# jhuldr/BrainFM

Measured on AMD Instinct MI355X. Metric: voxels/sec whole-volume multi-task inference, 256^3 tiled, higher is better.
Workload: dtype f16x3-split (fp32-grade); 1 GPU; 256^3 volume, reference tiling win160/stride80 -> 27 tiles, UNet3D f64 x6 levels, 9 heads (69 ch), fused tail + deformed atlas + on-device stitch of 17 keys; stitched_keys=17, mfma_passes=3, submission=hipGraph replay per tile shape, parallelism=tiles sharded over 1 rank(s), gather to rank 0, tiles_in_flight_per_gpu=2

## Files before the change

### brainfm_amd/_lib.py

```python
import ctypes as C
import os

_HERE = os.path.dirname(os.path.abspath(__file__))
LIB_PATH = os.path.join(_HERE, "libbrainfm_hip.so")

ERR = {0: "BFM_OK", -1: "BFM_E_ARG", -2: "BFM_E_SHAPE", -3: "BFM_E_WORKSPACE", -4: "BFM_E_LAUNCH"}

ROLE_PLAIN, ROLE_CT, ROLE_BIAS_LOG, ROLE_SEG, ROLE_DIST, ROLE_SR, ROLE_PATHOL = range(7)
(EW_EXP, EW_AFFINE, EW_CLAMP, EW_CLAMP_MIN, EW_GAMMA, EW_SIGMOID, EW_DIV, EW_NONZERO, EW_SUB_DIV, EW_GE,
 EW_NAN_TO_NUM) = range(11)
(EW_ADD, EW_MUL, EW_MUL_EXP, EW_AXPY_CLAMP0, EW_AXPY, EW_DIV2, EW_ZERO_WHERE_ZERO) = range(7)


class BfmError(RuntimeError):
    pass


class Upsample(C.Structure):
    _fields_ = [("d", C.c_int), ("h", C.c_int), ("w", C.c_int),
                ("mapD", C.c_void_p), ("mapH", C.c_void_p), ("mapW", C.c_void_p),
                ("repD", C.c_void_p), ("repH", C.c_void_p), ("repW", C.c_void_p)]


CLASS_STATS_BLOCKS = 1024


class TailDesc(C.Structure):
    _fields_ = [("n_out", C.c_int), ("c_feat", C.c_int),
                ("head_w", C.c_void_p), ("head_b", C.c_void_p), ("roles", C.c_void_p), ("out_slot", C.c_void_p),
                ("seg_first", C.c_int), ("n_seg", C.c_int), ("seg_lut", C.c_void_p),
                ("n_dist", C.c_int), ("dist_first", C.c_int), ("max_dist", C.c_float),
                ("unit_feat", C.c_int), ("slot_high_res", C.c_int), ("slot_fake_cortical", C.c_int),
                ("n_maps", C.c_int), ("head_wmax", C.c_float), ("skip_zero_input", C.c_int)]


class ZoomAxis(C.Structure):
    _fields_ = [("f", C.c_void_p), ("c", C.c_void_p), ("wf", C.c_void_p), ("wc", C.c_void_p)]


class KSet(C.Structure):
    _fields_ = [("k", C.c_void_p * 7), ("coef", C.c_float * 7), ("nk", C.c_int)]


class Dopri5Advect(C.Structure):
    _fields_ = [("y", C.c_void_p * 2), ("f", C.c_void_p * 2), ("k", C.c_void_p * 5),
                ("Vx", C.c_void_p), ("Vy", C.c_void_p), ("Vz", C.c_void_p),
                ("sx", C.c_int), ("sy", C.c_int), ("sz", C.c_int), ("neumann_bc", C.c_int), ("is_f64", C.c_int),
                ("atol", C.c_double), ("rtol", C.c_double), ("tol_min_dt", C.c_double), ("dt_max", C.c_double),
                ("safety", C.c_double), ("ifactor", C.c_double), ("dfactor", C.c_double),
                ("t_out", C.c_void_p), ("nt", C.c_int), ("sol", C.c_void_p), ("state", C.c_void_p),
                ("workspace", C.c_void_p)]


class AgeParams(C.Structure):
    _fields_ = [(n, C.c_void_p) for n in ("c1w", "c1b", "c2w", "c2b", "l1w", "l1b", "l2w", "l2b", "l3w", "l3b")]


class AgeGrads(C.Structure):
    _fields_ = [(n, C.c_void_p) for n in ("c1w", "c1b", "c2w", "c2b", "l1w", "l1b", "l2w", "l2b", "l3w", "l3b")]


GATHER_MAX_JOBS = 12


VERTEX_SETS_MAX = 4


class VertexSet(C.Structure):
    _fields_ = [("V", C.c_void_p), ("n", C.c_int64)]


class GatherJob(C.Structure):
    _fields_ = [("src", C.c_void_p), ("out", C.c_void_p), ("mean", C.c_float), ("scale", C.c_float), ("pre", C.c_int),
                ("default_max", C.c_int), ("post_div", C.c_float), ("clamp", C.c_int), ("clamp_lo", C.c_float),
                ("clamp_hi", C.c_float), ("sign", C.c_float), ("want_minmax", C.c_int)]


_P = C.c_void_p
_I = C.c_int
_F = C.c_float
_L = C.c_int64
_Z = C.c_size_t
_UP = C.POINTER(Upsample)

SIGNATURES = {
    "bfm_version": (C.c_char_p, []),
    "bfm_gn_stats_workspace": (_Z, [_I, _I, _I, _I, _I, _UP]),
    "bfm_gn_stats": (_I, [_P, _I, _P, _I, _I, _I, _I, _UP, _P, _P, _I, _F, _P, _P, _P, _P, _Z, _P]),
    "bfm_pack_conv_weights_direct": (_I, [_P, _I, _I, _P, _P]),
    "bfm_pack_conv_weights_mfma_bytes": (_Z, [_I, _I]),
    "bfm_pack_conv_weights_mfma": (_I, [_P, _I, _I, _F, _P, C.POINTER(_I), _P]),
    "bfm_pack_conv_weights_mfma16_bytes": (_Z, [_I, _I]),
    "bfm_pack_conv_weights_mfma16": (_I, [_P, _I, _I, _F, _P, C.POINTER(_I), _P]),
    "bfm_conv3x3x3_direct": (_I, [_P, _I, _P, _I, _I, _I, _I, _UP, _P, _P, _P, _I, _F, _P, _P]),
    "bfm_pack_conv_weights_upfold_bytes": (C.c_size_t, [_I, _I, _I]),
    "bfm_pack_conv_weights_upfold": (_I, [_P, _I, _I, _I, _F, _I, _P, _P, _P]),
    "bfm_conv3x3x3_upfold": (_I, [_P, _I, _I, _I, _I, _P, _P, _P, _I, _P, _I, _I, _I, _P, _P]),
    "bfm_conv3x3x3_upfold_workspace": (_Z, [_I, _I, _I, _I, _I]),
    "bfm_conv3x3x3_upfold_ex": (_I, [_P, _I, _I, _I, _I, _P, _P, _P, _I, _P, _I, _I, _I, _P, _P, _Z, _P]),
    "bfm_conv3x3x3_upfold_batch_workspace": (_Z, [_I, _I, _I, _I, _I, _I]),
    "bfm_conv3x3x3_upfold_batch": (_I, [_P, _I, _I, _I, _I, _I, _P, _P, _P, _I, _P, _I, _I, _I, _P, _P, _Z, _I, _P]),
    "bfm_moment_rows_bytes": (_Z, [_I, _I]),
    "bfm_conv3x3x3_mfma_rows": (_I, [_I, _I, _I, _I, _I, C.POINTER(_I)]),
    "bfm_conv3x3x3_mfma_ex": (_I, [_P, _I, _P, _I, _I, _I, _I, _UP, _P, _P, _P, _I, _P, _I, _I, _F, _I,
                                   C.POINTER(_I), _P, _P, _Z, _P, _P]),
    "bfm_conv3x3x3_mfma_batch_workspace": (_Z, [_I, _I, _I, _I, _I, _I, _I]),
    "bfm_conv3x3x3_mfma_batch": (_I, [_P, _I, _P, _I, _I, _I, _I, _I, _UP, _P, _P, _P, _I, _P, _I, _I, _F, _I,
                                      C.POINTER(_I), _P, _P, _Z, _P, _I, _P]),
    "bfm_gn_stats_batch_workspace": (_Z, [_I, _I, _I, _I, _I, _I, _UP]),
    "bfm_gn_stats_batch": (_I, [_P, _I, _P, _I, _I, _I, _I, _I, _UP, _P, _P, _I, _F, _P, _P, _P, _P, _Z, _P]),
    "bfm_gn_stats_rows_batch": (_I, [_P, _I, _I, _P, _I, _I, C.c_double, _L, _I, _P, _P, _I, _F, _P, _P, _P, _P]),
    "bfm_conv3x3x3_stem_rows": (_I, [_I, _I, _I]),
    "bfm_conv3x3x3_stem_ex": (_I, [_P, _I, _I, _I, _P, _P, _P, _P, _I, _F, _P, _P, _P]),
    "bfm_conv3x3x3_stem_mc_ex": (_I, [_P, _I, _I, _I, _I, _P, _P, _P, _P, _I, _F, _P, _P, _P]),
    "bfm_gn_stats_rows_workspace": (_Z, [_I, _I, _I, _I]),
    "bfm_gn_stats_rows": (_I, [_P, _I, _I, _P, _I, _I, C.c_double, _L, _P, _P, _I, _F, _P, _P, _P, _P, _Z, _P, _P]),
    "bfm_gn_stats_rows_sliced": (_I, [_P, _I, _I, _I, _I, _P, _I, _I, _I, _I, C.c_double, _L, _P, _P, _I, _F, _P, _P, _P, _P, _Z,
                                      _P, _P]),
    "bfm_gn_stats_rows_train": (_I, [_P, _I, _I, _P, _I, _I, C.c_double, _L, _P, _P, _I, _F, _P, _P, _P, _P, _P, _P, _Z, _P, _P]),
    "bfm_crop3d": (_I, [_P, _I, _I, _I, _I, _I, _I, _I, _I, _I, _P, _P]),
    "bfm_pack_conv_weights_wino4_bytes": (_Z, [_I, _I, _I]),
    "bfm_pack_conv_weights_wino4": (_I, [_P, _I, _I, _F, _I, _P, C.POINTER(_I), _P]),
    "bfm_conv3x3x3_wino4_rows": (_I, [_I, _I, _I, _I]),
    "bfm_conv3x3x3_wino4_box": (_I, [_I, _I, _I, _I, _P]),
    "bfm_conv3x3x3_wino4_masked_workspace": (_Z, [_I, _I, _I, _I]),
    "bfm_conv3x3x3_wino4_uniform_scratch": (_Z, [_I]),
    "bfm_conv3x3x3_wino4_uniform": (_I, [_P, _I, _I, _I, _I, _P, _P, _P, _I, _P, _I, _I, _F, _I, _I, _P, _P, _P, _P, _P]),
    "bfm_conv3x3x3_wino4": (_I, [_P, _I, _I, _I, _I, _P, _P, _P, _I, _P, _I, _I, _F, _I, _I, _P, _P, _P]),
    "bfm_conv3x3x3_wino4_batch": (_I, [_P, _I, _I, _I, _I, _I, _P, _P, _P, _I, _P, _I, _I, _F, _I, _I, _P, _P, _I, _P]),
    "bfm_conv3x3x3_wino4_masked": (_I, [_P, _I, _I, _I, _I, _P, _P, _P, _I, _P, _I, _I, _F, _I, _I, _P, _P, _P, _Z, _P]),
    "bfm_permute_flip3d": (_I, [_P, _I, _I, _I, C.POINTER(_I), C.POINTER(_I), _P, _P]),
    "bfm_bbox_nonzero": (_I, [_P, _I, _I, _I, _F, _P, _P]),
    "bfm_mean_lastdim": (_I, [_P, _L, _I, _P, _P]),
    "bfm_pack_conv_weights_wino_bytes": (_Z, [_I, _I, _I]),
    "bfm_pack_conv_weights_wino": (_I, [_P, _I, _I, _F, _I, _P, C.POINTER(_I), _P]),
    "bfm_bspline3_prefilter_axis": (_I, [_P, _I, _I, _I, _I, _I, _F, _F, _P, _F, _F, _F, _P]),
    "bfm_bspline3_resample_axis": (_I, [_P, _I, _I, _I, _I, _P, _I, _I, _P, _P]),
    "bfm_conv3x3x3_wino_rows": (_I, [_I, _I, _I, _I]),
    "bfm_conv3x3x3_wino_ex": (_I, [_P, _I, _I, _I, _I, _P, _P, _P, _I, _P, _I, _I, _F, _I, _I, _P, _P, _P]),
    "bfm_conv3x3x3_wino_box": (_I, [_I, _I, _I, _I, _P]),
    "bfm_uniform_boxes": (_I, [_P, _I, _I, _I, _I, _I, _P, _P]),
    "bfm_uniform_boxes_level": (_I, [_P, _I, _I, _I, _I, _I, _I, _P, _P]),
    "bfm_uniform_boxes_bytes": (_Z, [_I, _I, _I, _I]),
    "bfm_conv3x3x3_wino_uniform_scratch": (_Z, [_I]),
    "bfm_conv3x3x3_wino_uniform": (_I, [_P, _I, _I, _I, _I, _P, _P, _P, _I, _P, _I, _I, _F, _I, _I, _P, _P, _P, _P, _P]),
    "bfm_conv3x3x3_wino_pool_ok": (_I, [_I, _I, _I, _I]),
    "bfm_conv3x3x3_wino_pool": (_I, [_P, _I, _I, _I, _I, _P, _P, _P, _I, _P, _I, _I, _F, _I, _I, _P, _P, _P, _P, _P]),
    "bfm_conv3x3x3_wino_uniform_pool": (_I, [_P, _I, _I, _I, _I, _P, _P, _P, _I, _P, _I, _I, _F, _I, _I, _P, _P, _P, _P, _P, _P,
                                             _P]),
    "bfm_conv3x3x3_wino_masked_workspace": (_Z, [_I, _I, _I, _I]),
    "bfm_conv3x3x3_wino_masked": (_I, [_P, _I, _I, _I, _I, _P, _P, _P, _I, _P, _I, _I, _F, _I, _I, _P, _P, _P, _Z, _P]),
    "bfm_maxpool2_rows": (_I, [_I, _I, _I, _I]),
    "bfm_maxpool2_ex": (_I, [_P, _I, _I, _I, _I, _P, _P, _P]),
    "bfm_maxpool2_batch_rows": (_I, [_I, _I, _I, _I]),
    "bfm_maxpool2_batch": (_I, [_P, _I, _I, _I, _I, _I, _P, _P, _P]),
    "bfm_grid_push3d_linear": (_I, [_P, _I, _I, _I, _I, _I, _P, _I, _I, _I, _I, C.POINTER(_I), _I, _P, _P]),
    "bfm_grid_grad3d_linear": (_I, [_P, _I, _I, _I, _I, _I, _P, _I, _I, _I, _I, C.POINTER(_I), _I, _P, _P]),
    "bfm_gn_stats_train": (_I, [_P, _I, _P, _I, _I, _I, _I, _UP, _P, _P, _I, _F, _P, _P, _P, _P, _P, _P, _Z, _P]),
    "bfm_lrelu_bwd": (_I, [_P, _P, _L, _F, _P, _P]),
    "bfm_lrelu_bwd_ex": (_I, [_P, _P, _L, _F, _P, _P, _P]),
    "bfm_conv3x3x3_wgrad_workspace": (_Z, [_I, _I, _I, _I, _I]),
    "bfm_conv3x3x3_wgrad": (_I, [_P, _I, _P, _I, _P, _I, _I, _I, _I, _UP, _P, _P, _P, _P, _Z, _P]),
    "bfm_conv3x3x3_wgrad_ex": (_I, [_P, _I, _P, _I, _P, _I, _I, _I, _I, _UP, _P, _P, _P, _P, _I, _I, _P, _P, _Z, _P]),
    "bfm_stem_mc_bwd_workspace": (_Z, [_I, _I, _I, _I, _I]),
    "bfm_stem_mc_bwd": (_I, [_P, _I, _P, _I, _I, _I, _I, _P, _P, _P, _P, _P, _P, _P, _P, _P, _Z, _P]),
    "bfm_gn_bwd_workspace": (_Z, [_I, _I, _I, _I]),
    "bfm_gn_bwd": (_I, [_P, _P, _I, _P, _I, _I, _I, _I, _UP, _P, _P, _P, _P, _P, _P, _I, _P, _P, _P, _P, _P, _Z, _P]),
    "bfm_maxpool2_bwd": (_I, [_P, _P, _I, _I, _I, _I, _P, _P]),
    "bfm_transpose_mirror_weights": (_I, [_P, _I, _I, _I, _P, _P]),
    "bfm_loss_workspace": (_Z, [_I]),
    "bfm_loss_l1": (_I, [_P, _I, _I, _P, _P, _P, _L, _F, _I, _F, _P, _P, _P, _Z, _P]),
    "bfm_loss_l1_multi_workspace": (_Z, []),
    "bfm_loss_l1_multi": (_I, [_P, _I, _L, _I, _P, _P, _P, _P, _P, _P, _P, _P, _P, _P, _Z, _P]),
    "bfm_loss_grad_l1_multi": (_I, [_P, _I, _I, _P, _P, _P, _P, _I, _I, _I, _P, _P, _P, _Z, _P]),
    "bfm_loss_grad_l1": (_I, [_P, _I, _I, _P, _P, _I, _I, _I, _F, _P, _P, _P, _Z, _P]),
    "bfm_loss_seg": (_I, [_P, _I, _I, _I, _P, _P, _P, _L, _F, _F, _P, _P, _P, _P, _Z, _P]),
    "bfm_loss_pathol_workspace": (_Z, []),
    "bfm_loss_pathol": (_I, [_P, _L, _L, _P, _L, _F, _F, _P, _P, _P, _P, _Z, _P]),
    "bfm_loss_reg_workspace": (_Z, [_I, _I, _I, _I]),
    "bfm_loss_reg_smooth": (_I, [_P, _L, _L, _L, _I, _I, _I, _I, _F, _P, _P, _P, _Z, _P]),
    "bfm_loss_reg_hessian": (_I, [_P, _L, _L, _L, _I, _I, _I, _I, _F, _P, _P, _P, _Z, _P]),
    "bfm_loss_contrastive_workspace": (_Z, []),
    "bfm_loss_contrastive": (_I, [_P, _P, _I, _L, _I, _F, _F, _F, _F, _F, _P, _P, _P, _P, _P, _P, _Z, _P]),
    "bfm_head_bwd_workspace": (_Z, [_I, _I, _L]),
    "bfm_head_bwd": (_I, [_P, _P, _P, _I, _I, _L, _P, _P, _P, _P, _Z, _P]),
    "bfm_tail_raw_rows": (_I, [_P, _L, C.POINTER(TailDesc), _P, _P, _L, _P]),
    "bfm_loss_l1_multi_rows": (_I, [_P, _L, _I, _L, _I, _P, _P, _P, _P, _P, _P, _P, _P, _P, _P, _Z, _P]),
    "bfm_loss_grad_l1_multi_rows": (_I, [_P, _L, _I, _I, _P, _P, _P, _P, _I, _I, _I, _P, _P, _P, _Z, _P]),
    "bfm_loss_seg_rows": (_I, [_P, _L, _I, _I, _I, _P, _P, _P, _L, _F, _F, _P, _P, _P, _P, _Z, _P]),
    "bfm_head_bwd_rows": (_I, [_P, _L, _P, _P, _I, _I, _L, _P, _P, _P, _P, _Z, _P]),
    "bfm_normalize_bwd": (_I, [_P, _P, _I, _L, _F, _P, _P]),
    "bfm_adamw_step": (_I, [_P, _P, _P, _P, _L, _F, _F, _F, _F, _F, _I, _F, _P]),
    "bfm_grad_sumsq": (_I, [_P, _L, _P, _P, _P, _Z, _P]),
    "bfm_grad_sumsq_multi": (_I, [_P, _I, _P, _I, _L, _P, _P, _P, _Z, _P]),
    "bfm_adamw_step_multi": (_I, [_P, _I, _P, _I, _L, _F, _F, _F, _F, _F, _P]),
    "bfm_conv3x3x3_mfma_workspace": (_Z, [_I, _I, _I, _I, _I, _I]),
    "bfm_conv3x3x3_mfma_plan": (_I, [_I, _I, _I, _I, _I, C.POINTER(_I)]),
    "bfm_conv3x3x3_mfma": (_I, [_P, _I, _P, _I, _I, _I, _I, _UP, _P, _P, _P, _I, _P, _I, _I, _F, _I,
                                C.POINTER(_I), _P, _P, _Z, _P]),
    "bfm_maxpool2": (_I, [_P, _I, _I, _I, _I, _P, _P]),
    "bfm_tail_heads": (_I, [_P, _P, _L, C.POINTER(TailDesc), _P, _P, _P, _P, _P, _P]),
    "bfm_tail_heads_rows": (_I, [_P, _P, _L, C.POINTER(TailDesc), _P, _P, _L, _P, _P, _I, _P]),
    "bfm_ew_unary": (_I, [_I, _P, _L, _P, _L, _L, _F, _F, _P]),
    "bfm_ew_binary": (_I, [_I, _P, _L, _P, _L, _P, _L, _L, _F, _P]),
    "bfm_absmax_f32": (_I, [_P, _L, _L, _L, _P, _P]),
    "bfm_softmax_cl": (_I, [_P, _L, _I, _P, _L, _L, _P]),
    "bfm_argmax_lut_cl": (_I, [_P, _L, _I, _P, _P, _L, _P]),
    "bfm_fake_cortical": (_I, [_P, _L, _I, _P, _L, _P]),
    "bfm_mask_concat2": (_I, [_P, _P, _L, _P, _P]),
    "bfm_condition_input": (_I, [_P, _P, _I, _I, _I, _I, _P, _P, _P, _P]),
    "bfm_interp3d_linear": (_I, [_P, _I, _I, _I, _I, _P, _P, _P, _L, _F, _P, _P]),
    "bfm_interp3d_nearest": (_I, [_P, _I, _I, _I, _I, _P, _P, _P, _L, _P, _P]),
    "bfm_deformed_atlas": (_I, [_P, _P, _P, _P, _P, _I, _I, _I, C.POINTER(_F), _L, _P, _P]),
    "bfm_deformed_atlas_tile": (_I, [_P, _P, _P, _P, _P, _I, _I, _I, C.POINTER(_F), _L, _P, _P]),
    "bfm_zoom_linear": (_I, [_P, _I, _I, _I, _I, C.POINTER(ZoomAxis), _I, _I, _I, _P, _P]),
    "bfm_conv1d_axis": (_I, [_P, _I, _I, _I, _I, _P, _I, _P, _P]),
    "bfm_grid_pull3d_linear": (_I, [_P, _I, _I, _I, _I, _I, _P, _I, _I, _I, _I, C.POINTER(_I), _I, _P, _P]),
    "bfm_deform_grid_workspace": (_Z, [_I, _I, _I]),
    "bfm_deform_grid": (_I, [_P, _I, _I, _I, C.POINTER(_F), C.POINTER(_F), C.POINTER(_I), _P, _P, _P, _P, _P, _Z, _P]),
    "bfm_label_gauss": (_I, [_P, _P, _P, _P, _L, _I, _P, _P]),
    "bfm_label_class_stats": (_I, [_P, _P, _L, _P, _P, _P, _P]),
    "bfm_onehot_lut": (_I, [_P, _P, _I, _I, _L, _P, _P]),
    "bfm_perlin3d": (_I, [_P, _I, _I, _I, _I, _I, _I, _P, _P]),
    "bfm_radix_hist_f64": (_I, [_P, _L, C.c_uint64, _I, _P, _P]),
    "bfm_threshold_mask_f64": (_I, [_P, _L, C.c_double, _P, _P, _P]),
    "bfm_curl3d": (_I, [_P, _P, _P, _I, _I, _I, _F, _P, _P, _P, _P]),
    "bfm_advect_upwind_rhs": (_I, [_P, _I, _P, _P, _P, _I, _I, _I, _I, _P, _P]),
    "bfm_rk_combine": (_I, [_P, _I, C.POINTER(KSet), _P, _L, _P]),
    "bfm_reduce_workspace": (_Z, []),
    "bfm_rk_error_sumsq": (_I, [C.POINTER(KSet), _P, _P, _I, C.c_double, C.c_double, _L, _P, _P, _Z, _P]),
    "bfm_scaled_sumsq": (_I, [_P, _P, _I, _P, _I, C.c_double, C.c_double, _L, _P, _P, _Z, _P]),
    "bfm_dopri5_dense_eval": (_I, [_P, _P, _I, C.POINTER(KSet), C.c_double, C.c_double, _P, _L, _P]),
    "bfm_reduce_f32": (_I, [_I, _P, _P, _L, _P, _P, _Z, _P]),
    "bfm_reduce_f64": (_I, [_I, _P, _P, _L, _P, _P, _Z, _P]),
    "bfm_dopri5_advect_state_bytes": (_Z, []),
    "bfm_dopri5_advect_workspace": (_Z, [_I, _I, _I]),
    "bfm_dopri5_advect_init": (_I, [C.POINTER(Dopri5Advect), C.c_double, C.c_double, _P]),
    "bfm_dopri5_advect_steps": (_I, [C.POINTER(Dopri5Advect), _I, _P]),
    "bfm_randn_philox": (_I, [_P, _L, C.c_uint64, C.c_uint64, _F, _P]),
    "bfm_svf_integrate_workspace": (_Z, [_I, _I, _I]),
    "bfm_svf_integrate": (_I, [_P, _I, _I, _I, _I, _P, _P, _P, _Z, _P]),
    "bfm_deform_vertices": (_I, [_P, _I, _I, _I, C.POINTER(VertexSet), _I, C.POINTER(_F), C.POINTER(_F), _I, _I, _P]),
    "bfm_deform_zoom_workspace": (_Z, []),
    "bfm_deform_zoom_minmax": (_I, [_P, _I, _I, _I, C.POINTER(ZoomAxis), _I, _I, _I, _I, C.POINTER(_F), C.POINTER(_F),
                                    C.POINTER(_I), _P, _P, _Z, _P]),
    "bfm_deform_zoom_write": (_I, [_P, _I, _I, _I, C.POINTER(ZoomAxis), _I, _I, _I, _I, C.POINTER(_F), C.POINTER(_F),
                                   C.POINTER(_I), C.POINTER(_F), _P, _P, _P, _P, _P]),
    "bfm_gather_targets_workspace": (_Z, []),
    "bfm_gather_targets": (_I, [C.POINTER(GatherJob), _I, _I, _I, _I, C.POINTER(_I), _P, _P, _P, _I, _I, _I, _I, _P, _P,
                                _Z, _P]),
    "bfm_minmax_normalise": (_I, [_P, _L, _P, _P]),
    "bfm_gather_onehot": (_I, [_P, _I, _I, _I, C.POINTER(_I), _P, _P, _P, _I, _I, _I, _I, _P, _I, _I, _P, _P, _P]),
    "bfm_gather_onehot_rows": (_I, [_P, _I, _I, _I, C.POINTER(_I), _P, _P, _P, _I, _I, _I, _I, _P, _I, _I, _P, _P, _P]),
    "bfm_percentile_workspace": (_Z, []),
    "bfm_percentile_f64": (_I, [_P, _L, _L, _I, C.c_double, _P, _P, _Z, _P]),
    "bfm_shape_workspace": (_Z, []),
    "bfm_shape_threshold_f64": (_I, [_P, _L, _P, _P, _P, _P, _P, _Z, _P]),
    "bfm_shape_binarize": (_I, [_P, _I, _L, _P, C.c_double, _P, _P, _P, _Z, _P]),
    "bfm_pathology_mask": (_I, [_P, _P, _I, _P, _L, _P, _P, _Z, _P]),
    "bfm_pathology_encode_workspace": (_Z, []),
    "bfm_pathology_encode_dev": (_I, [_P, _P, _P, _I, _P, C.POINTER(_F), _I, _P, _L, _P, _P, _P, _Z, _P]),
    "bfm_interp3d_linear_axes": (_I, [_P, _I, _I, _I, _P, _P, _P, _I, _I, _I, _F, _P, _P]),
    "bfm_sample_finalize": (_I, [_P, _P, _I, _I, _I, _P, _I, _P, _P, _P]),
    "bfm_stitch_accumulate": (_I, [_P, _P, _P, _I, _I, _I, _P, _I, _I, _I, _I, _I, _I, _P]),
    "bfm_stitch_accumulate_multi": (_I, [_P, _L, _P, _I, _P, _P, _I, _I, _I, _P, _I, _I, _I, _I, _I, _I, _P]),
    "bfm_tile_count_add": (_I, [_P, _I, _I, _I, _I, _I, _I, _I, _I, _I, _P]),
    "bfm_pack_tile_multi": (_I, [_P, _L, _P, _I, _P, _P, _L, _P, _P]),
    "bfm_divide_by_count_multi": (_I, [_P, _P, _L, _I, _P]),
    "bfm_stitch_gather_multi": (_I, [_P, _I, _I, _P, _I, _I, _I, _P]),
    "bfm_tile_mask_blocks": (_I, [_L]),
    "bfm_tile_mask_index": (_I, [_P, _I, _I, _I, _P, _I, _I, _P, _P, _P, _P]),
    "bfm_pack_tile_compact": (_I, [_P, _L, _P, _I, _P, _P, _L, _P, _L, _P, _P]),
    "bfm_stitch_gather_compact": (_I, [_P, _I, _I, _P, _P, _I, _I, _I, _P]),
    "bfm_maxpool4": (_I, [_P, _I, _I, _I, _I, _P, _P, _P]),
    "bfm_maxpool4_bwd": (_I, [_P, _P, _I, _I, _I, _I, _P, _I, _P]),
    "bfm_age_conv_fwd": (_I, [_P, _I, _I, _I, _I, _P, _P, _I, _P, _P]),
    "bfm_age_conv_bwd_workspace": (_Z, [_I, _I, _I, _I, _I]),
    "bfm_age_conv_bwd": (_I, [_P, _I, _I, _I, _I, _P, _I, _P, _P, _P, _P, _P, _P, _Z, _P]),
    "bfm_age_mlp_fwd": (_I, [_P, _I, C.POINTER(AgeParams), _I, _P, _P, _P, _P]),
    "bfm_age_mlp_bwd_workspace": (_Z, []),
    "bfm_age_mlp_bwd": (_I, [_P, _I, C.POINTER(AgeParams), _I, _P, _P, _P, _P, C.c_double, _F, _P, C.POINTER(AgeGrads),
                             _P, _P, _Z, _P]),
}

_lib = None


def register(sigs):
    SIGNATURES.update(sigs)
    if _lib is not None:
        _bind(_lib, sigs)


def _bind(lib, sigs):
    for name, (res, args) in sigs.items():
        try:
            fn = getattr(lib, name)
        except AttributeError as e:
            raise BfmError("libbrainfm_hip.so does not export %s -- rebuild it" % name) from e
        fn.restype = res
        fn.argtypes = args


def load():
    global _lib
    if _lib is None:
        if not os.path.exists(LIB_PATH):
            raise BfmError("HIP extension missing: %s (run `python -m brainfm_amd.build`); "
                           "there is no CPU fallback in the product path" % LIB_PATH)
        import torch
        lib = C.CDLL(LIB_PATH)
        _bind(lib, SIGNATURES)
        _lib = lib
    return _lib


def check(rc, what):
    if rc != 0:
        raise BfmError("%s failed: %s (%d)" % (what, ERR.get(rc, "?"), rc))


def ptr(t):
    if t is None:
        return None
    return C.c_void_p(t.data_ptr())


def stream_ptr():
    import torch
    raw = getattr(torch._C, "_cuda_getCurrentRawStream", None)
    if raw is not None:
        return C.c_void_p(raw(torch._C._cuda_getDevice()))
    return C.c_void_p(torch.cuda.current_stream().cuda_stream)


def on_device(pick):
    import functools

    def deco(fn):
        @functools.wraps(fn)
        def wrapped(*a, **k):
            import torch
            d = pick(*a, **k)
            if isinstance(d, torch.Tensor):
                d = d.device
            if isinstance(d, int):
                d = torch.device("cuda", d)
            if isinstance(d, str):
                d = torch.device(d)
            if d is None or d.type != "cuda" or d.index is None or d.index == torch.cuda.current_device():
                return fn(*a, **k)
            with torch.cuda.device(d):
                return fn(*a, **k)
        return wrapped
    return deco
```

### brainfm_amd/csrc/conv3d_mfma.hip

```cpp
#include "conv_shared.h"
#include <cstdlib>
#include <type_traits>

namespace {

typedef _Float16 half8 __attribute__((ext_vector_type(8)));
typedef _Float16 half4 __attribute__((ext_vector_type(4)));
typedef float floatx16 __attribute__((ext_vector_type(16)));

constexpr int KC = 16;
#ifdef BFM_STAMPS
__device__ long long g_stamps[4096];
#define STAMP(i) do { if (stamp_on) g_stamps[stamp_base + (i)] = clock64(); } while (0)
#else
#define STAMP(i) do {} while (0)
#endif
constexpr int FRAG_U4 = 64;

struct ConvParams {
    const float *A, *B;
    int CA, CB, D, H, W;
    UpView up;
    const float *scale, *shift, *bound;
    int G;
    const uint4* wp;
    int wexp;
    int Cout;
    float slope;
    float* out;
    int TD, TH, TW, HT, WT;
    int nTy, nTx, nMt, NT;
    int KCN, kc_per_split, splitk;
    int nvox_lds, plane_stride;
    int tw_shift, thw_shift;
    int64_t split_stride;
    int accum;
    int S, nMtS;
    int saff;
    int64_t sA, sB, sO;
    double *rsum, *rsq;
    float *rmn, *rmx;
    int abl;
};


template <int WM, int WN>
__device__ __forceinline__ void store_moment_row(const ConvParams& p, unsigned char* lds, int tid, int wm, int wn,
                                                 bool writer, const int (&col)[4], int ncol, const double (&s)[4],
                                                 const double (&q)[4], const float (&mn)[4], const float (&mx)[4],
                                                 int mt, int nt) {
    double* ls = reinterpret_cast<double*>(lds);
    double* lq = ls + WM * WN * 64;
    float* lmn = reinterpret_cast<float*>(lq + WM * WN * 64);
    float* lmx = lmn + WM * WN * 64;
    __syncthreads();
    if (writer) {
#pragma unroll
        for (int j = 0; j < 4; ++j) {
            if (j < ncol) {
                const int i = (wm * WN + wn) * 64 + col[j];
                ls[i] = s[j]; lq[i] = q[j]; lmn[i] = mn[j]; lmx[i] = mx[j];
            }
        }
    }
    __syncthreads();
    if (tid < 64 * WN) {
        const int w2 = tid >> 6, c = tid & 63;
        double S = 0.0, Q = 0.0;
        float MN = INFINITY, MX = -INFINITY;
#pragma unroll
        for (int m = 0; m < WM; ++m) {
            const int i = (m * WN + w2) * 64 + c;
            S += ls[i]; Q += lq[i];
            MN = fminf(MN, lmn[i]); MX = fmaxf(MX, lmx[i]);
        }
        const size_t o = (size_t)mt * p.Cout + (nt * WN + w2) * 64 + c;
        p.rsum[o] = S; p.rsq[o] = Q; p.rmn[o] = MN; p.rmx[o] = MX;
    }
}

__device__ __forceinline__ void box_coords(const ConvParams& p, int q, int& d, int& h, int& w) {
    if (p.tw_shift >= 0 && p.thw_shift >= 0) {
        d = q >> p.thw_shift;
        int rem = q & ((1 << p.thw_shift) - 1);
        h = rem >> p.tw_shift;
        w = rem & ((1 << p.tw_shift) - 1);
    } else {
        int thw = p.TH * p.TW;
        d = q / thw;
        int rem = q - d * thw;
        h = rem / p.TW;
        w = rem - h * p.TW;
    }
}

template <int ROWS, int NTHR>
__device__ __forceinline__ const int* build_row_table(const ConvParams& p, unsigned char* lds, int tid, int z0, int y0, int x0,
                                                      int boxN) {
    int* tab = reinterpret_cast<int*>(lds);
    for (int q = tid; q < ROWS; q += NTHR) {
        int rel = -1;
        if (q < boxN) {
            int d, h, w;
            box_coords(p, q, d, h, w);
            if (z0 + d < p.D && y0 + h < p.H && x0 + w < p.W) rel = ((d * p.H + h) * p.W + w) * p.Cout;
        }
        tab[q] = rel;
    }
    return tab;
}

template <int WM, int WN, int NPASS, int NSLOT>
__global__ void __launch_bounds__(64 * WM * WN, 2) conv_mfma(const ConvParams p) {
    constexpr int NTHR = 64 * WM * WN;
    constexpr int NW = WM * WN;
    constexpr int NPL = (NPASS == 3) ? 2 : 1;
    constexpr int ROWFR = 12 * WN;
    constexpr int KPR = ROWFR / NW;
    constexpr int DPF = NSLOT - 1;
    static_assert(ROWFR % NW == 0, "row fragments must split evenly over the waves");
    extern __shared__ __attribute__((aligned(16))) unsigned char lds[];

    const int tid = threadIdx.x;
    const int lane = tid & 63;
    const int wave = __builtin_amdgcn_readfirstlane(tid >> 6);
    const int wm = wave / WN, wn = wave % WN;
    const int l32 = lane & 31, khalf = lane >> 5;

    int bid = blockIdx.x;
    {
        const int nblk = p.nMt * p.NT;
        const int q = nblk >> 3, r = nblk & 7;
        const int xcd = bid & 7, idx = bid >> 3;
        bid = (xcd < r ? xcd * (q + 1) : r * (q + 1) + (xcd - r) * q) + idx;
    }
    int mt, nt, smp = 0;
    if (p.S > 1) {
        smp = bid % p.S;
        const int t = bid / p.S;
        nt = t % p.NT;
        mt = smp * p.nMtS + t / p.NT;
    } else {
        mt = bid / p.NT;
        nt = bid - mt * p.NT;
    }
    const int mtl = mt - smp * p.nMtS;
    const float* const pA = p.A + smp * p.sA;
    const float* const pB = p.B + smp * p.sB;
    const float* const pscale = p.scale + smp * p.saff;
    const float* const pshift = p.shift + smp * p.saff;
    const float* const pbound = p.bound + smp * p.G;
    float* const pout = p.out + smp * p.sO;
    const int split = blockIdx.y;
#ifdef BFM_STAMPS
    const bool stamp_on = tid == 0 && (blockIdx.x == 0 || blockIdx.x == gridDim.x / 2 + 3) && blockIdx.y == gridDim.y / 2;
    int stamp_base = blockIdx.x == 0 ? 0 : 1024;
    long long t_wait = 0, t_bar = 0;
#endif
    const int tx = mtl % p.nTx;
    const int ty = (mtl / p.nTx) % p.nTy;
    const int tz = mtl / (p.nTx * p.nTy);
    const int z0 = tz * p.TD, y0 = ty * p.TH, x0 = tx * p.TW;
    const int boxN = p.TD * p.TH * p.TW;

    float bmax = 0.f;
    for (int g = 0; g < p.G; ++g) bmax = fmaxf(bmax, pbound[g]);
    int aexp = 0;
    if (bmax > 0.f && bmax < INFINITY) {
        int ex;
        (void)frexpf(bmax, &ex);
        aexp = 14 - ex;
        aexp = aexp > 60 ? 60 : (aexp < -60 ? -60 : aexp);
    }
    const float a_scale = ldexpf(1.0f, aexp);
    const float dq = ldexpf(1.0f, -(aexp + p.wexp));

    int a_off[2];
#pragma unroll
    for (int mb = 0; mb < 2; ++mb) {
        int q = wm * 64 + mb * 32 + row_perm(l32);
        int d = 0, h = 0, w = 0;
        if (q < boxN) box_coords(p, q, d, h, w);
        int vox = (d * p.HT + h) * p.WT + w;
        a_off[mb] = (khalf * NPL) * p.plane_stride + vox * 16;
    }

    constexpr int MAX_IT = 12;
    const int n_el = p.nvox_lds * 4;
    const int q4 = tid & 3;
    int off[MAX_IT];
    auto compute_offsets = [&](bool fromB) {
#pragma unroll
        for (int it = 0; it < MAX_IT; ++it) {
            const int e = tid + it * NTHR;
            off[it] = -2;
            if (e < n_el) {
                const int vox = e >> 2;
                const int hz = vox / (p.HT * p.WT);
                const int rem = vox - hz * (p.HT * p.WT);
                const int hy = rem / p.WT;
                const int hx = rem - hy * p.WT;
                const int gz = z0 + hz - 1, gy = y0 + hy - 1, gx = x0 + hx - 1;
                off[it] = -1;
                if (gz >= 0 && gz < p.D && gy >= 0 && gy < p.H && gx >= 0 && gx < p.W) {
                    if (fromB) off[it] = ((p.up.mapD[gz] * p.up.h + p.up.mapH[gy]) * p.up.w + p.up.mapW[gx]) * p.CB;
                    else off[it] = ((gz * p.H + gy) * p.W + gx) * p.CA;
                }
            }
        }
    };
    bool off_fromB = (split * p.kc_per_split * KC) >= p.CA;
    compute_offsets(off_fromB);
    const int st_plane = ((q4 >> 1) * NPL) * p.plane_stride + (q4 & 1) * 8;

    floatx16 acc[2][2];
#pragma unroll
    for (int mb = 0; mb < 2; ++mb)
#pragma unroll
        for (int nb = 0; nb < 2; ++nb)
#pragma unroll
            for (int i = 0; i < 16; ++i) acc[mb][nb][i] = 0.f;

    const int ntw = nt * WN + wn;
    if (p.accum && p.splitk == 1) {
        const float inv_dq = ldexpf(1.0f, aexp + p.wexp);
        const int* rowtab = build_row_table<WM * 64, NTHR>(p, lds, tid, z0, y0, x0, boxN);
        __syncthreads();
        const float* ib = pout + (((int64_t)z0 * p.H + y0) * p.W + x0) * p.Cout + ntw * 64 + l32;
#pragma unroll
        for (int mb = 0; mb < 2; ++mb) {
#pragma unroll
            for (int ig = 0; ig < 4; ++ig) {
                const int4 r4 = *reinterpret_cast<const int4*>(rowtab + wm * 64 + mb * 32 + row_perm(ig * 8 + khalf * 4));
                const int rel[4] = {r4.x, r4.y, r4.z, r4.w};
#pragma unroll
                for (int j = 0; j < 4; ++j) {
                    if (rel[j] < 0) continue;
                    const float* orow = ib + (unsigned)rel[j];
#pragma unroll
                    for (int nb = 0; nb < 2; ++nb) acc[mb][nb][ig * 4 + j] = orow[nb * 32] * inv_dq;
                }
            }
        }
    }
    const int kc_begin = split * p.kc_per_split;
    int kc_end = min(p.KCN, kc_begin + p.kc_per_split);
#ifdef BFM_MFMA_ABLATE
    if (p.abl & 32) kc_end = kc_begin;
#endif

    const int b_base = 2 * NPL * p.plane_stride;
    const int total_rows = (kc_end - kc_begin) * 9;
    auto issue_row = [&](int R) {
        const int Rc = R < total_rows ? R : total_rows - 1;
        const int kcR = kc_begin + Rc / 9, rr = Rc % 9;
        const int slot = R % NSLOT;
#pragma unroll
        for (int i = 0; i < KPR; ++i) {
            const int f = wave + i * NW;
            const int j = f / 12, g = f - j * 12;
            const uint4* src = p.wp + ((size_t)((nt * WN + j) * p.KCN + kcR) * 27 + rr * 3) * (4 * FRAG_U4) +
                               g * FRAG_U4 + lane;
            __builtin_amdgcn_global_load_lds((const __attribute__((address_space(1))) void*)src,
                                             (__attribute__((address_space(3))) void*)(lds + b_base +
                                                                                      (slot * ROWFR + f) * 1024),
                                             16, 0, 0);
        }
    };
    if (total_rows > 0) {
#pragma unroll
        for (int R = 0; R < DPF; ++R) issue_row(R);
    }

    for (int kc = kc_begin; kc < kc_end; ++kc) {
        const int c0 = kc * KC;
        const bool fromB = c0 >= p.CA;
        if (fromB != off_fromB) { off_fromB = fromB; compute_offsets(fromB); }
        const float* src = (fromB ? pB + (c0 - p.CA) : pA + c0) + q4 * 4;
        const float4 sc4 = *reinterpret_cast<const float4*>(pscale + c0 + q4 * 4);
        const float4 sh4 = *reinterpret_cast<const float4*>(pshift + c0 + q4 * 4);
        const float sc[4] = {sc4.x * a_scale, sc4.y * a_scale, sc4.z * a_scale, sc4.w * a_scale};
        const float sh[4] = {sh4.x * a_scale, sh4.y * a_scale, sh4.z * a_scale, sh4.w * a_scale};

        STAMP((kc - kc_begin) * 8 + 0);
        __syncthreads();
        STAMP((kc - kc_begin) * 8 + 1);
#pragma unroll
        for (int it0 = 0; it0 < MAX_IT; it0 += 4) {
            float4 v[4];
#pragma unroll
            for (int u = 0; u < 4; ++u) {
                v[u] = make_float4(0.f, 0.f, 0.f, 0.f);
                if (off[it0 + u] >= 0) v[u] = *reinterpret_cast<const float4*>(src + off[it0 + u]);
            }
#pragma unroll
            for (int u = 0; u < 4; ++u) {
                const int e = tid + (it0 + u) * NTHR;
                if (off[it0 + u] != -2) {
                    const bool ok = off[it0 + u] >= 0;
                    float y[4] = {v[u].x, v[u].y, v[u].z, v[u].w};
                    half4 hi, lo;
#pragma unroll
                    for (int i = 0; i < 4; ++i) {
                        float t = ok ? fmaf(y[i], sc[i], sh[i]) : 0.f;
                        _Float16 hh = (_Float16)t;
                        hi[i] = hh;
                        lo[i] = (_Float16)(t - (float)hh);
                    }
                    unsigned char* dst = lds + st_plane + (e >> 2) * 16;
                    *reinterpret_cast<half4*>(dst) = hi;
                    if constexpr (NPASS == 3) *reinterpret_cast<half4*>(dst + p.plane_stride) = lo;
                }
            }
        }
        STAMP((kc - kc_begin) * 8 + 2);
        __syncthreads();
        STAMP((kc - kc_begin) * 8 + 3);

        const int rbase = (kc - kc_begin) * 9;
        for (int r = 0; r < 9; ++r) {
            const int R = rbase + r;
#ifdef BFM_STAMPS
            long long ta = 0, tb = 0, tc = 0;
            if (stamp_on) ta = clock64();
#endif
            asm volatile("s_waitcnt vmcnt(%0)" ::"n"(KPR * (DPF - 1)) : "memory");
#ifdef BFM_STAMPS
            if (stamp_on) tb = clock64();
#endif
            __builtin_amdgcn_s_barrier();
#ifdef BFM_STAMPS
            if (stamp_on) { tc = clock64(); t_wait += tb - ta; t_bar += tc - tb; }
#endif
            issue_row(R + DPF);
            const unsigned char* bs = lds + b_base + ((R % NSLOT) * ROWFR + wn * 12) * 1024 + lane * 16;
            const int kd = r / 3, kh = r - kd * 3;
            const int roff = (kd * p.HT + kh) * p.WT * 16;
#pragma unroll
            for (int kw = 0; kw < 3; ++kw) {
                half8 a[2][NPL], b[2][NPL];
#pragma unroll
                for (int nb = 0; nb < 2; ++nb)
#pragma unroll
                    for (int hl = 0; hl < NPL; ++hl)
                        b[nb][hl] = *reinterpret_cast<const half8*>(bs + (kw * 4 + nb * 2 + hl) * 1024);
#pragma unroll
                for (int mb = 0; mb < 2; ++mb)
#pragma unroll
                    for (int hl = 0; hl < NPL; ++hl)
                        a[mb][hl] = *reinterpret_cast<const half8*>(lds + a_off[mb] + hl * p.plane_stride + roff +
                                                                    kw * 16);
#pragma unroll
                for (int mb = 0; mb < 2; ++mb)
#pragma unroll
                    for (int nb = 0; nb < 2; ++nb) {
                        if constexpr (NPASS == 3) {
                            acc[mb][nb] = __builtin_amdgcn_mfma_f32_32x32x16_f16(a[mb][1], b[nb][0], acc[mb][nb], 0, 0, 0);
                            acc[mb][nb] = __builtin_amdgcn_mfma_f32_32x32x16_f16(a[mb][0], b[nb][1], acc[mb][nb], 0, 0, 0);
                        }
                        acc[mb][nb] = __builtin_amdgcn_mfma_f32_32x32x16_f16(a[mb][0], b[nb][0], acc[mb][nb], 0, 0, 0);
                    }
            }
        }
    }
    asm volatile("s_waitcnt vmcnt(0)" ::: "memory");
#ifdef BFM_STAMPS
    if (stamp_on) { g_stamps[stamp_base + 1000] = t_wait; g_stamps[stamp_base + 1001] = t_bar; g_stamps[stamp_base + 1002] = clock64();
                    g_stamps[stamp_base + 1003] = kc_end - kc_begin; }
#endif

#ifdef BFM_MFMA_ABLATE
    if (p.abl & 16) {
        float sm = 0.f;
#pragma unroll
        for (int mb = 0; mb < 2; ++mb)
#pragma unroll
            for (int i = 0; i < 16; ++i) sm += acc[mb][0][i] + acc[mb][1][i];
        if (sm == 12345.678f) pout[tid] = sm;
        return;
    }
#endif
    const bool final_out = p.splitk == 1;
    const bool want_rows = final_out && p.rsum != nullptr;
    float* obase = pout + (final_out ? 0 : (int64_t)split * p.split_stride);
    float fs[4] = {0.f, 0.f, 0.f, 0.f}, fq[4] = {0.f, 0.f, 0.f, 0.f};
    float mmn[4] = {INFINITY, INFINITY, INFINITY, INFINITY}, mmx[4] = {-INFINITY, -INFINITY, -INFINITY, -INFINITY};
    __syncthreads();
    const int* rowtab = build_row_table<WM * 64, NTHR>(p, lds, tid, z0, y0, x0, boxN);
    __syncthreads();
    float* const ob = obase + (((int64_t)z0 * p.H + y0) * p.W + x0) * p.Cout + ntw * 64 + l32;
#pragma unroll
    for (int mb = 0; mb < 2; ++mb) {
#pragma unroll
        for (int ig = 0; ig < 4; ++ig) {
            const int4 r4 = *reinterpret_cast<const int4*>(rowtab + wm * 64 + mb * 32 + row_perm(ig * 8 + khalf * 4));
            const int rel[4] = {r4.x, r4.y, r4.z, r4.w};
#pragma unroll
            for (int j = 0; j < 4; ++j) {
                if (rel[j] < 0) continue;
                float* orow = ob + (unsigned)rel[j];
#pragma unroll
                for (int nb = 0; nb < 2; ++nb) {
                    float r = acc[mb][nb][ig * 4 + j] * dq;
                    if (final_out) r = r >= 0.f ? r : r * p.slope;
                    orow[nb * 32] = r;
                    if (want_rows) {
                        fs[nb] += r; fq[nb] = fmaf(r, r, fq[nb]);
                        mmn[nb] = fminf(mmn[nb], r); mmx[nb] = fmaxf(mmx[nb], r);
                    }
                }
            }
        }
    }
    if (want_rows) {
        double ms[4], mq[4];
#pragma unroll
        for (int j = 0; j < 4; ++j) { ms[j] = (double)fs[j]; mq[j] = (double)fq[j]; }
#pragma unroll
        for (int nb = 0; nb < 2; ++nb) {
            ms[nb] += __shfl_xor(ms[nb], 32);
            mq[nb] += __shfl_xor(mq[nb], 32);
            mmn[nb] = fminf(mmn[nb], __shfl_xor(mmn[nb], 32));
            mmx[nb] = fmaxf(mmx[nb], __shfl_xor(mmx[nb], 32));
        }
        const int cols[4] = {l32, 32 + l32, 0, 0};
        store_moment_row<WM, WN>(p, lds, tid, wm, wn, khalf == 0, cols, 2, ms, mq, mmn, mmx, mt, nt);
    }
}

template <int WM, int WN, int NPASS, int SP, int NSLOT>
__global__ void __launch_bounds__(64 * WM * WN, 2) conv_mfma16(const ConvParams p) {
    constexpr int NTHR = 64 * WM * WN;
    constexpr int NW = WM * WN;
    constexpr int NPL = (NPASS == 3) ? 2 : 1;
    constexpr int PAIRFR = 8 * WN;
    constexpr int SLOTFR = SP * PAIRFR;
    constexpr int KPS = SLOTFR / NW;
    constexpr int NSL = 14 / SP;
    constexpr int DPF = NSLOT - 1;
    static_assert(SLOTFR % NW == 0 && 14 % SP == 0, "slot geometry");
    typedef float floatx4 __attribute__((ext_vector_type(4)));
    extern __shared__ __attribute__((aligned(16))) unsigned char lds[];

    const int tid = threadIdx.x;
    const int lane = tid & 63;
    const int wave = __builtin_amdgcn_readfirstlane(tid >> 6);
    const int wm = wave / WN, wn = wave % WN;
    const int l16 = lane & 15, kg = lane >> 4;

    int bid = blockIdx.x;
    {
        const int nblk = p.nMt * p.NT;
        const int q = nblk >> 3, r = nblk & 7;
        const int xcd = bid & 7, idx = bid >> 3;
        bid = (xcd < r ? xcd * (q + 1) : r * (q + 1) + (xcd - r) * q) + idx;
    }
    int mt, nt, smp = 0;
    if (p.S > 1) {
        smp = bid % p.S;
        const int t = bid / p.S;
        nt = t % p.NT;
        mt = smp * p.nMtS + t / p.NT;
    } else {
        mt = bid / p.NT;
        nt = bid - mt * p.NT;
    }
    const int mtl = mt - smp * p.nMtS;
    const float* const pA = p.A + smp * p.sA;
    const float* const pB = p.B + smp * p.sB;
    const float* const pscale = p.scale + smp * p.saff;
    const float* const pshift = p.shift + smp * p.saff;
    const float* const pbound = p.bound + smp * p.G;
    float* const pout = p.out + smp * p.sO;
    const int split = blockIdx.y;
    const int tx = mtl % p.nTx;
    const int ty = (mtl / p.nTx) % p.nTy;
    const int tz = mtl / (p.nTx * p.nTy);
    const int z0 = tz * p.TD, y0 = ty * p.TH, x0 = tx * p.TW;
    const int boxN = p.TD * p.TH * p.TW;

    float bmax = 0.f;
    for (int g = 0; g < p.G; ++g) bmax = fmaxf(bmax, pbound[g]);
    int aexp = 0;
    if (bmax > 0.f && bmax < INFINITY) {
        int ex;
        (void)frexpf(bmax, &ex);
        aexp = 14 - ex;
        aexp = aexp > 60 ? 60 : (aexp < -60 ? -60 : aexp);
    }
    const float a_scale = ldexpf(1.0f, aexp);
    const float dq = ldexpf(1.0f, -(aexp + p.wexp));

    int a_off[4];
#pragma unroll
    for (int rb = 0; rb < 4; ++rb) {
        int q = wm * 64 + rb * 16 + l16;
        int d = 0, h = 0, w = 0;
        if (q < boxN) box_coords(p, q, d, h, w);
        int vox = (d * p.HT + h) * p.WT + w;
        a_off[rb] = ((kg & 1) * NPL) * p.plane_stride + vox * 16;
    }

    constexpr int MAX_IT = 12;
    const int n_el = p.nvox_lds * 4;
    const int q4 = tid & 3;
    int off[MAX_IT];
    auto compute_offsets = [&](bool fromB) __attribute__((always_inline)) {
#pragma unroll
        for (int it = 0; it < MAX_IT; ++it) {
            const int e = tid + it * NTHR;
            off[it] = -2;
            if (e < n_el) {
                const int vox = e >> 2;
                const int hz = vox / (p.HT * p.WT);
                const int rem = vox - hz * (p.HT * p.WT);
                const int hy = rem / p.WT;
                const int hx = rem - hy * p.WT;
                const int gz = z0 + hz - 1, gy = y0 + hy - 1, gx = x0 + hx - 1;
                off[it] = -1;
                if (gz >= 0 && gz < p.D && gy >= 0 && gy < p.H && gx >= 0 && gx < p.W) {
                    if (fromB) off[it] = ((p.up.mapD[gz] * p.up.h + p.up.mapH[gy]) * p.up.w + p.up.mapW[gx]) * p.CB;
                    else off[it] = ((gz * p.H + gy) * p.W + gx) * p.CA;
                }
            }
        }
    };
    bool off_fromB = (split * p.kc_per_split * KC) >= p.CA;
    compute_offsets(off_fromB);
    const int st_plane = ((q4 >> 1) * NPL) * p.plane_stride + (q4 & 1) * 8;

    floatx4 acc[4][4];
#pragma unroll
    for (int rb = 0; rb < 4; ++rb)
#pragma unroll
        for (int cb = 0; cb < 4; ++cb)
#pragma unroll
            for (int i = 0; i < 4; ++i) acc[rb][cb][i] = 0.f;

    const int ntw = nt * WN + wn;
    if (p.accum && p.splitk == 1) {
        const float inv_dq = ldexpf(1.0f, aexp + p.wexp);
        const int* rowtab = build_row_table<WM * 64, NTHR>(p, lds, tid, z0, y0, x0, boxN);
        __syncthreads();
        const float* ib = pout + (((int64_t)z0 * p.H + y0) * p.W + x0) * p.Cout + ntw * 64 + l16;
#pragma unroll
        for (int rb = 0; rb < 4; ++rb) {
            const int4 r4 = *reinterpret_cast<const int4*>(rowtab + wm * 64 + rb * 16 + kg * 4);
            const int rel[4] = {r4.x, r4.y, r4.z, r4.w};
#pragma unroll
            for (int i = 0; i < 4; ++i) {
                if (rel[i] < 0) continue;
                const float* orow = ib + (unsigned)rel[i];
#pragma unroll
                for (int cb = 0; cb < 4; ++cb) acc[rb][cb][i] = orow[cb * 16] * inv_dq;
            }
        }
    }
    const int kc_begin = split * p.kc_per_split;
    int kc_end = min(p.KCN, kc_begin + p.kc_per_split);
#ifdef BFM_MFMA_ABLATE
    if (p.abl & 32) kc_end = kc_begin;
#endif
    const int b_base = 2 * NPL * p.plane_stride;
    const int total_slots = (kc_end - kc_begin) * NSL;
    auto issue_slot = [&](int S) __attribute__((always_inline)) {
        const int Sc = S < total_slots ? S : total_slots - 1;
        const int kcS = kc_begin + Sc / NSL, sl = Sc % NSL;
        const int slot = S % NSLOT;
#pragma unroll
        for (int i = 0; i < KPS; ++i) {
            const int f = wave + i * NW;
            const int j = f / (SP * 8), rem = f - j * (SP * 8);
            const int pr = rem >> 3, g = rem & 7;
            const uint4* src = p.wp + ((size_t)((nt * WN + j) * p.KCN + kcS) * 14 + sl * SP + pr) * (8 * FRAG_U4) +
                               g * FRAG_U4 + lane;
            __builtin_amdgcn_global_load_lds((const __attribute__((address_space(1))) void*)src,
                                             (__attribute__((address_space(3))) void*)(lds + b_base +
                                                                                      (slot * SLOTFR + f) * 1024),
                                             16, 0, 0);
        }
    };
    if (total_slots > 0) {
#pragma unroll
        for (int S = 0; S < DPF; ++S) issue_slot(S);
    }

    for (int kc = kc_begin; kc < kc_end; ++kc) {
        const int c0 = kc * KC;
        const bool fromB = c0 >= p.CA;
        if (fromB != off_fromB) { off_fromB = fromB; compute_offsets(fromB); }
        const float* src = (fromB ? pB + (c0 - p.CA) : pA + c0) + q4 * 4;
        const float4 sc4 = *reinterpret_cast<const float4*>(pscale + c0 + q4 * 4);
        const float4 sh4 = *reinterpret_cast<const float4*>(pshift + c0 + q4 * 4);
        const float sc[4] = {sc4.x * a_scale, sc4.y * a_scale, sc4.z * a_scale, sc4.w * a_scale};
        const float sh[4] = {sh4.x * a_scale, sh4.y * a_scale, sh4.z * a_scale, sh4.w * a_scale};

        __syncthreads();
#pragma unroll
        for (int it0 = 0; it0 < MAX_IT; it0 += 4) {
            float4 v[4];
#pragma unroll
            for (int u = 0; u < 4; ++u) {
                v[u] = make_float4(0.f, 0.f, 0.f, 0.f);
                if (off[it0 + u] >= 0) v[u] = *reinterpret_cast<const float4*>(src + off[it0 + u]);
            }
#pragma unroll
            for (int u = 0; u < 4; ++u) {
                const int e = tid + (it0 + u) * NTHR;
                if (off[it0 + u] != -2) {
                    const bool ok = off[it0 + u] >= 0;
                    float y[4] = {v[u].x, v[u].y, v[u].z, v[u].w};
                    half4 hi, lo;
#pragma unroll
                    for (int i = 0; i < 4; ++i) {
                        float t = ok ? fmaf(y[i], sc[i], sh[i]) : 0.f;
                        _Float16 hh = (_Float16)t;
                        hi[i] = hh;
                        lo[i] = (_Float16)(t - (float)hh);
                    }
                    unsigned char* dst = lds + st_plane + (e >> 2) * 16;
                    *reinterpret_cast<half4*>(dst) = hi;
                    if constexpr (NPASS == 3) *reinterpret_cast<half4*>(dst + p.plane_stride) = lo;
                }
            }
        }
        __syncthreads();

        const int sbase = (kc - kc_begin) * NSL;
        for (int sl = 0; sl < NSL; ++sl) {
            const int S = sbase + sl;
            asm volatile("s_waitcnt vmcnt(%0)" ::"n"(KPS * (DPF - 1)) : "memory");
            __builtin_amdgcn_s_barrier();
            issue_slot(S + DPF);
#pragma unroll
            for (int pr = 0; pr < SP; ++pr) {
                const int P = sl * SP + pr;
                const int t0 = 2 * P, t1 = min(2 * P + 1, 26);
                const int kd0 = t0 / 9, r0 = t0 - kd0 * 9, kh0 = r0 / 3, kw0 = r0 - kh0 * 3;
                const int kd1 = t1 / 9, r1 = t1 - kd1 * 9, kh1 = r1 / 3, kw1 = r1 - kh1 * 3;
                const int toff0 = ((kd0 * p.HT + kh0) * p.WT + kw0) * 16;
                const int toff1 = ((kd1 * p.HT + kh1) * p.WT + kw1) * 16;
                const int toff = (kg >> 1) ? toff1 : toff0;
                const unsigned char* bs = lds + b_base + ((S % NSLOT) * SLOTFR + (wn * SP + pr) * 8) * 1024 + lane * 16;
                half8 a[4][NPL], b[4][NPL];
#pragma unroll
                for (int cb = 0; cb < 4; ++cb)
#pragma unroll
                    for (int hl = 0; hl < NPL; ++hl)
                        b[cb][hl] = *reinterpret_cast<const half8*>(bs + (cb * 2 + hl) * 1024);
#pragma unroll
                for (int rb = 0; rb < 4; ++rb)
#pragma unroll
                    for (int hl = 0; hl < NPL; ++hl)
                        a[rb][hl] = *reinterpret_cast<const half8*>(lds + a_off[rb] + hl * p.plane_stride + toff);
#pragma unroll
                for (int rb = 0; rb < 4; ++rb)
#pragma unroll
                    for (int cb = 0; cb < 4; ++cb) {
                        if constexpr (NPASS == 3) {
                            acc[rb][cb] = __builtin_amdgcn_mfma_f32_16x16x32_f16(a[rb][1], b[cb][0], acc[rb][cb], 0, 0, 0);
                            acc[rb][cb] = __builtin_amdgcn_mfma_f32_16x16x32_f16(a[rb][0], b[cb][1], acc[rb][cb], 0, 0, 0);
                        }
                        acc[rb][cb] = __builtin_amdgcn_mfma_f32_16x16x32_f16(a[rb][0], b[cb][0], acc[rb][cb], 0, 0, 0);
                    }
            }
        }
    }
    asm volatile("s_waitcnt vmcnt(0)" ::: "memory");

#ifdef BFM_MFMA_ABLATE
    if (p.abl & 16) {
        float sm = 0.f;
#pragma unroll
        for (int rb = 0; rb < 4; ++rb)
#pragma unroll
            for (int cb = 0; cb < 4; ++cb) sm += acc[rb][cb][0] + acc[rb][cb][1] + acc[rb][cb][2] + acc[rb][cb][3];
        if (sm == 12345.678f) pout[tid] = sm;
        return;
    }
#endif
    const bool final_out = p.splitk == 1;
    const bool want_rows = final_out && p.rsum != nullptr;
    float* obase = pout + (final_out ? 0 : (int64_t)split * p.split_stride);
    float fs[4] = {0.f, 0.f, 0.f, 0.f}, fq[4] = {0.f, 0.f, 0.f, 0.f};
    float mmn[4] = {INFINITY, INFINITY, INFINITY, INFINITY}, mmx[4] = {-INFINITY, -INFINITY, -INFINITY, -INFINITY};
    __syncthreads();
    const int* rowtab = build_row_table<WM * 64, NTHR>(p, lds, tid, z0, y0, x0, boxN);
    __syncthreads();
    float* const ob = obase + (((int64_t)z0 * p.H + y0) * p.W + x0) * p.Cout + ntw * 64 + l16;
#pragma unroll
    for (int rb = 0; rb < 4; ++rb) {
        const int4 r4 = *reinterpret_cast<const int4*>(rowtab + wm * 64 + rb * 16 + kg * 4);
        const int rel[4] = {r4.x, r4.y, r4.z, r4.w};
#pragma unroll
        for (int i = 0; i < 4; ++i) {
            if (rel[i] < 0) continue;
            float* orow = ob + (unsigned)rel[i];
#pragma unroll
            for (int cb = 0; cb < 4; ++cb) {
                float r = acc[rb][cb][i] * dq;
                if (final_out) r = r >= 0.f ? r : r * p.slope;
                orow[cb * 16] = r;
                if (want_rows) {
                    fs[cb] += r; fq[cb] = fmaf(r, r, fq[cb]);
                    mmn[cb] = fminf(mmn[cb], r); mmx[cb] = fmaxf(mmx[cb], r);
                }
            }
        }
    }
    if (want_rows) {
        double ms[4], mq[4];
#pragma unroll
        for (int j = 0; j < 4; ++j) { ms[j] = (double)fs[j]; mq[j] = (double)fq[j]; }
#pragma unroll
        for (int cb = 0; cb < 4; ++cb) {
#pragma unroll
            for (int m = 16; m <= 32; m <<= 1) {
                ms[cb] += __shfl_xor(ms[cb], m);
                mq[cb] += __shfl_xor(mq[cb], m);
                mmn[cb] = fminf(mmn[cb], __shfl_xor(mmn[cb], m));
                mmx[cb] = fmaxf(mmx[cb], __shfl_xor(mmx[cb], m));
            }
        }
        const int cols[4] = {l16, 16 + l16, 32 + l16, 48 + l16};
        store_moment_row<WM, WN>(p, lds, tid, wm, wn, kg == 0, cols, 4, ms, mq, mmn, mmx, mt, nt);
    }
}

__global__ void pack_mfma16(const float* __restrict__ w, int Cin, int Cout, int wexp, uint4* __restrict__ out) {
    const int KCN = Cin / KC;
    const int64_t n = (int64_t)(Cout / 64) * KCN * 14 * 4 * 2 * 64;
    const float s = ldexpf(1.0f, wexp);
    for (int64_t i = (int64_t)blockIdx.x * blockDim.x + threadIdx.x; i < n; i += (int64_t)gridDim.x * blockDim.x) {
        int lane = (int)(i & 63);
        int64_t r = i >> 6;
        int hl = (int)(r & 1); r >>= 1;
        int cb = (int)(r & 3); r >>= 2;
        int pair = (int)(r % 14); r /= 14;
        int kc = (int)(r % KCN);
        int ntile = (int)(r / KCN);
        int co = ntile * 64 + cb * 16 + (lane & 15);
        int kgq = lane >> 4;
        int tap = 2 * pair + (kgq >> 1);
        int ci0 = kc * KC + (kgq & 1) * 8;
        half8 v;
#pragma unroll
        for (int j = 0; j < 8; ++j) {
            float x = tap < 27 ? w[((int64_t)co * Cin + ci0 + j) * 27 + tap] * s : 0.f;
            _Float16 hh = (_Float16)x;
            v[j] = hl ? (_Float16)(x - (float)hh) : hh;
        }
        out[i] = *reinterpret_cast<uint4*>(&v);
    }
}

constexpr int PK16_ROW = KC * 27 + 1;
__global__ void __launch_bounds__(256) pack_mfma16_tiled(const float* __restrict__ w, int Cin, int Cout, int wexp,
                                                         uint4* __restrict__ out) {
    extern __shared__ float pk16_lds[];
    const int KCN = Cin / KC;
    const int half = blockIdx.x & 1;
    const int kc = (blockIdx.x >> 1) % KCN, ntile = (blockIdx.x >> 1) / KCN;
    const float s = ldexpf(1.0f, wexp);
    const float* src0 = w + ((int64_t)(ntile * 64 + half * 32) * Cin + kc * KC) * 27;
    bfm_stage_rows<32, KC * 27, PK16_ROW, 256>(src0, (int64_t)Cin * 27, pk16_lds, s,
                                               ((reinterpret_cast<uintptr_t>(w) & 15) == 0) && (Cin & 3) == 0);
    __syncthreads();
    uint4* dst = out + (int64_t)(blockIdx.x >> 1) * (14 * 4 * 2 * 64);
    const int lane = threadIdx.x & 63, wave = threadIdx.x >> 6;
    const int kgq = lane >> 4;
    for (int q = wave; q < 14 * 2; q += 4) {
        const int cbl = q & 1, pair = q >> 1;
        const int tap = 2 * pair + (kgq >> 1);
        const float* src = pk16_lds + (cbl * 16 + (lane & 15)) * PK16_ROW + ((kgq & 1) * 8) * 27 + min(tap, 26);
        half8 vh, vl;
#pragma unroll
        for (int j = 0; j < 8; ++j) {
            const float x = tap < 27 ? src[j * 27] : 0.f;
            const _Float16 hh = (_Float16)x;
            vh[j] = hh;
            vl[j] = (_Float16)(x - (float)hh);
        }
        dst[((pair * 4 + half * 2 + cbl) * 2 + 0) * 64 + lane] = *reinterpret_cast<uint4*>(&vh);
        dst[((pair * 4 + half * 2 + cbl) * 2 + 1) * 64 + lane] = *reinterpret_cast<uint4*>(&vl);
    }
}

__device__ __forceinline__ void ws_tile_coords(const ConvParams& p, int lin, int& mt, int& nt) {
    const int nblk = p.nMt * p.NT;
    const int q = nblk >> 3, r = nblk & 7;
    const int xcd = lin & 7, idx = lin >> 3;
    const int bid = (xcd < r ? xcd * (q + 1) : r * (q + 1) + (xcd - r) * q) + idx;
    mt = bid / p.NT;
    nt = bid - mt * p.NT;
}

template <int WM, int WN, int NPASS>
__global__ void __launch_bounds__(512, 2) conv_mfma_ws(const ConvParams p) {
    constexpr int NPL = (NPASS == 3) ? 2 : 1;
    constexpr int ROWFR = 12 * WN;
    constexpr int KPR = ROWFR / 4;
    constexpr int PTHR = 256;
    extern __shared__ __attribute__((aligned(16))) unsigned char lds[];

    const int tid = threadIdx.x;
    const int lane = tid & 63;
    const int wave = __builtin_amdgcn_readfirstlane(tid >> 6);
    const bool producer = wave >= 4;
    const int split = blockIdx.y;
    const int boxN = p.TD * p.TH * p.TW;
    const int ntiles = p.nMt * p.NT;
    const int G = gridDim.x;
    const int my_tiles = (ntiles - (int)blockIdx.x + G - 1) / G;

    float bmax = 0.f;
    for (int g = 0; g < p.G; ++g) bmax = fmaxf(bmax, p.bound[g]);
    int aexp = 0;
    if (bmax > 0.f && bmax < INFINITY) {
        int ex;
        (void)frexpf(bmax, &ex);
        aexp = 14 - ex;
        aexp = aexp > 60 ? 60 : (aexp < -60 ? -60 : aexp);
    }
    const float a_scale = ldexpf(1.0f, aexp);
    const float dq = ldexpf(1.0f, -(aexp + p.wexp));

    const int a_bytes = 2 * NPL * p.plane_stride;
    const int b_base = 2 * a_bytes;
    const int kc_begin = split * p.kc_per_split;
    const int kc_end = min(p.KCN, kc_begin + p.kc_per_split);
    const int nchunks = kc_end - kc_begin;
    const int total_chunks = my_tiles * nchunks;
    const int total_rows = total_chunks * 9;
    if (total_chunks <= 0) return;

    if (producer) {
        const int ptid = tid - 256;
        const int pw = wave - 4;
        constexpr int MAX_IT = 12;
        const int n_el = p.nvox_lds * 4;
        const int q4 = ptid & 3;
        int off[MAX_IT];
        int z0 = 0, y0 = 0, x0 = 0;
        auto compute_offsets = [&](bool fromB) __attribute__((always_inline)) {
#pragma unroll
            for (int it = 0; it < MAX_IT; ++it) {
                const int e = ptid + it * PTHR;
                off[it] = -2;
                if (e < n_el) {
                    const int vox = e >> 2;
                    const int hz = vox / (p.HT * p.WT);
                    const int rem = vox - hz * (p.HT * p.WT);
                    const int hy = rem / p.WT;
                    const int hx = rem - hy * p.WT;
                    const int gz = z0 + hz - 1, gy = y0 + hy - 1, gx = x0 + hx - 1;
                    off[it] = -1;
                    if (gz >= 0 && gz < p.D && gy >= 0 && gy < p.H && gx >= 0 && gx < p.W) {
                        if (fromB) off[it] = ((p.up.mapD[gz] * p.up.h + p.up.mapH[gy]) * p.up.w + p.up.mapW[gx]) * p.CB;
                        else off[it] = ((gz * p.H + gy) * p.W + gx) * p.CA;
                    }
                }
            }
        };
        bool off_fromB = false;
        const int st_plane = ((q4 >> 1) * NPL) * p.plane_stride + (q4 & 1) * 8;

        float4 v[12];
        float sc[4], sh[4];
        const float* src = nullptr;
        auto begin_chunk = [&](int g) __attribute__((always_inline)) {
            const int c = g % nchunks;
            const int c0 = (kc_begin + c) * KC;
            const bool fromB = c0 >= p.CA;
            if (c == 0) {
                int mt, nt;
                ws_tile_coords(p, (int)blockIdx.x + (g / nchunks) * G, mt, nt);
                const int tx = mt % p.nTx;
                const int ty = (mt / p.nTx) % p.nTy;
                const int tz = mt / (p.nTx * p.nTy);
                z0 = tz * p.TD; y0 = ty * p.TH; x0 = tx * p.TW;
                off_fromB = fromB;
                compute_offsets(fromB);
            } else if (fromB != off_fromB) {
                off_fromB = fromB;
                compute_offsets(fromB);
            }
            src = (fromB ? p.B + (c0 - p.CA) : p.A + c0) + q4 * 4;
            const float4 sc4 = *reinterpret_cast<const float4*>(p.scale + c0 + q4 * 4);
            const float4 sh4 = *reinterpret_cast<const float4*>(p.shift + c0 + q4 * 4);
            sc[0] = sc4.x * a_scale; sc[1] = sc4.y * a_scale; sc[2] = sc4.z * a_scale; sc[3] = sc4.w * a_scale;
            sh[0] = sh4.x * a_scale; sh[1] = sh4.y * a_scale; sh[2] = sh4.z * a_scale; sh[3] = sh4.w * a_scale;
        };
        auto load_el = [&](auto itc) __attribute__((always_inline)) {
            constexpr int it = decltype(itc)::value;
            const int o = off[it] >= 0 ? off[it] : 0;
            v[it] = *reinterpret_cast<const float4*>(src + o);
        };
        auto write_el = [&](auto itc, int buf) __attribute__((always_inline)) {
            constexpr int it = decltype(itc)::value;
            const int o = off[it];
            const int e = ptid + it * PTHR;
            if (o != -2) {
                const bool ok = o >= 0;
                float y[4] = {v[it].x, v[it].y, v[it].z, v[it].w};
                half4 hi, lo;
#pragma unroll
                for (int i = 0; i < 4; ++i) {
                    float t = ok ? fmaf(y[i], sc[i], sh[i]) : 0.f;
                    _Float16 hh = (_Float16)t;
                    hi[i] = hh;
                    lo[i] = (_Float16)(t - (float)hh);
                }
                unsigned char* dst = lds + buf * a_bytes + st_plane + (e >> 2) * 16;
                *reinterpret_cast<half4*>(dst) = hi;
                if constexpr (NPASS == 3) *reinterpret_cast<half4*>(dst + p.plane_stride) = lo;
            }
        };
        auto issue_row = [&](int R) __attribute__((always_inline)) {
            const int Rs = R < total_rows ? R : total_rows - 1;
            const int g = Rs / 9, rr = Rs - g * 9;
            int mt, nt;
            ws_tile_coords(p, (int)blockIdx.x + (g / nchunks) * G, mt, nt);
            const int kcR = kc_begin + g % nchunks;
            const int slot = R % 3;
#pragma unroll
            for (int i = 0; i < KPR; ++i) {
                const int f = pw + i * 4;
                const int j = f / 12, gg = f - j * 12;
                const uint4* wsrc = p.wp + ((size_t)((nt * WN + j) * p.KCN + kcR) * 27 + rr * 3) * (4 * FRAG_U4) +
                                    gg * FRAG_U4 + lane;
                __builtin_amdgcn_global_load_lds((const __attribute__((address_space(1))) void*)wsrc,
                                                 (__attribute__((address_space(3))) void*)(lds + b_base +
                                                                                          (slot * ROWFR + f) * 1024),
                                                 16, 0, 0);
            }
        };
        auto for_el = [&](auto first, auto count, auto&& fn) __attribute__((always_inline)) {
            constexpr int f0 = decltype(first)::value, n = decltype(count)::value;
            if constexpr (n >= 1) fn(std::integral_constant<int, f0>{});
            if constexpr (n >= 2) fn(std::integral_constant<int, f0 + 1>{});
        };
#define BFM_IC(n) std::integral_constant<int, n>{}

        begin_chunk(0);
        for_el(BFM_IC(0), BFM_IC(2), [&](auto i) { load_el(i); });  for_el(BFM_IC(0), BFM_IC(2), [&](auto i) { write_el(i, 0); });
        for_el(BFM_IC(2), BFM_IC(2), [&](auto i) { load_el(i); });  for_el(BFM_IC(2), BFM_IC(2), [&](auto i) { write_el(i, 0); });
        for_el(BFM_IC(4), BFM_IC(2), [&](auto i) { load_el(i); });  for_el(BFM_IC(4), BFM_IC(2), [&](auto i) { write_el(i, 0); });
        for_el(BFM_IC(6), BFM_IC(2), [&](auto i) { load_el(i); });  for_el(BFM_IC(6), BFM_IC(2), [&](auto i) { write_el(i, 0); });
        for_el(BFM_IC(8), BFM_IC(2), [&](auto i) { load_el(i); });  for_el(BFM_IC(8), BFM_IC(2), [&](auto i) { write_el(i, 0); });
        for_el(BFM_IC(10), BFM_IC(2), [&](auto i) { load_el(i); }); for_el(BFM_IC(10), BFM_IC(2), [&](auto i) { write_el(i, 0); });
        issue_row(0);
        issue_row(1);
        asm volatile("s_waitcnt vmcnt(0) lgkmcnt(0)" ::: "memory");

        for (int g = 0; g < total_chunks; ++g) {
            const bool more = g + 1 < total_chunks;
            const int nbuf = (g + 1) & 1;
            if (more) begin_chunk(g + 1);
            auto row = [&](auto rc) __attribute__((always_inline)) {
                constexpr int r = decltype(rc)::value;
                constexpr int NL_PREV = r == 0 ? 0 : (r <= 4 ? 2 : 1);
                constexpr int NL = r <= 3 ? 2 : (r <= 7 ? 1 : 0);
                constexpr int F_PREV = r == 0 ? 0 : (r <= 4 ? 2 * (r - 1) : 8 + (r - 5));
                constexpr int F = r <= 3 ? 2 * r : 8 + (r - 4);
                const int R = g * 9 + r;
                if (more) asm volatile("s_waitcnt vmcnt(%0)" ::"n"(NL_PREV + KPR) : "memory");
                else asm volatile("s_waitcnt vmcnt(%0)" ::"n"(KPR) : "memory");
                asm volatile("s_waitcnt lgkmcnt(0)" ::: "memory");
                __builtin_amdgcn_s_barrier();
                if (more) {
                    for_el(BFM_IC(F_PREV), BFM_IC(NL_PREV), [&](auto i) { write_el(i, nbuf); });
                    for_el(BFM_IC(F), BFM_IC(NL), [&](auto i) { load_el(i); });
                }
                issue_row(R + 2);
            };
            row(BFM_IC(0)); row(BFM_IC(1)); row(BFM_IC(2)); row(BFM_IC(3)); row(BFM_IC(4));
            row(BFM_IC(5)); row(BFM_IC(6)); row(BFM_IC(7)); row(BFM_IC(8));
        }
#undef BFM_IC
        asm volatile("s_waitcnt vmcnt(0) lgkmcnt(0)" ::: "memory");
        return;
    }

    const int wm = wave / WN, wn = wave % WN;
    const int l32 = lane & 31, khalf = lane >> 5;
    int a_off[2];
#pragma unroll
    for (int mb = 0; mb < 2; ++mb) {
        int q = wm * 64 + mb * 32 + row_perm(l32);
        int d = 0, h = 0, w = 0;
        if (q < boxN) box_coords(p, q, d, h, w);
        int vox = (d * p.HT + h) * p.WT + w;
        a_off[mb] = (khalf * NPL) * p.plane_stride + vox * 16;
    }
    floatx16 acc[2][2];
    const bool final_out = p.splitk == 1;
    float* obase = p.out + (final_out ? 0 : (int64_t)split * p.split_stride);

    for (int g = 0; g < total_chunks; ++g) {
        const int c = g % nchunks;
        if (c == 0) {
#pragma unroll
            for (int mb = 0; mb < 2; ++mb)
#pragma unroll
                for (int nb = 0; nb < 2; ++nb)
#pragma unroll
                    for (int i = 0; i < 16; ++i) acc[mb][nb][i] = 0.f;
        }
        const unsigned char* abuf = lds + (g & 1) * a_bytes;
        for (int r = 0; r < 9; ++r) {
            const int R = g * 9 + r;
            __builtin_amdgcn_s_barrier();
            const unsigned char* bs = lds + b_base + ((R % 3) * ROWFR + wn * 12) * 1024 + lane * 16;
            const int kd = r / 3, kh = r - kd * 3;
            const int roff = (kd * p.HT + kh) * p.WT * 16;
#pragma unroll
            for (int kw = 0; kw < 3; ++kw) {
                half8 a[2][NPL], b[2][NPL];
#pragma unroll
                for (int nb = 0; nb < 2; ++nb)
#pragma unroll
                    for (int hl = 0; hl < NPL; ++hl)
                        b[nb][hl] = *reinterpret_cast<const half8*>(bs + (kw * 4 + nb * 2 + hl) * 1024);
#pragma unroll
                for (int mb = 0; mb < 2; ++mb)
#pragma unroll
                    for (int hl = 0; hl < NPL; ++hl)
                        a[mb][hl] = *reinterpret_cast<const half8*>(abuf + a_off[mb] + hl * p.plane_stride + roff +
                                                                    kw * 16);
#pragma unroll
                for (int mb = 0; mb < 2; ++mb)
#pragma unroll
                    for (int nb = 0; nb < 2; ++nb) {
                        if constexpr (NPASS == 3) {
                            acc[mb][nb] = __builtin_amdgcn_mfma_f32_32x32x16_f16(a[mb][1], b[nb][0], acc[mb][nb], 0, 0, 0);
                            acc[mb][nb] = __builtin_amdgcn_mfma_f32_32x32x16_f16(a[mb][0], b[nb][1], acc[mb][nb], 0, 0, 0);
                        }
                        acc[mb][nb] = __builtin_amdgcn_mfma_f32_32x32x16_f16(a[mb][0], b[nb][0], acc[mb][nb], 0, 0, 0);
                    }
            }
        }
        if (c == nchunks - 1) {
            int mt, nt;
            ws_tile_coords(p, (int)blockIdx.x + (g / nchunks) * G, mt, nt);
            const int tx = mt % p.nTx;
            const int ty = (mt / p.nTx) % p.nTy;
            const int tz = mt / (p.nTx * p.nTy);
            const int z0 = tz * p.TD, y0 = ty * p.TH, x0 = tx * p.TW;
            const int ntw = nt * WN + wn;
#pragma unroll
            for (int mb = 0; mb < 2; ++mb) {
#pragma unroll
                for (int i = 0; i < 16; ++i) {
                    const int rr = (i >> 2) * 8 + khalf * 4 + (i & 3);
                    const int q = wm * 64 + mb * 32 + row_perm(rr);
                    if (q >= boxN) continue;
                    int d, h, w;
                    box_coords(p, q, d, h, w);
                    const int gz = z0 + d, gy = y0 + h, gx = x0 + w;
                    if (gz >= p.D || gy >= p.H || gx >= p.W) continue;
                    float* orow = obase + (((int64_t)gz * p.H + gy) * p.W + gx) * p.Cout + ntw * 64 + l32;
#pragma unroll
                    for (int nb = 0; nb < 2; ++nb) {
                        float r = acc[mb][nb][i] * dq;
                        if (final_out) {
                            if (p.accum) r = r + orow[nb * 32];
                            r = r >= 0.f ? r : r * p.slope;
                        }
                        orow[nb * 32] = r;
                    }
                }
            }
        }
    }
}

__global__ void splitk_reduce(const float* __restrict__ ws, int splitk, int64_t n4, int64_t stride4, float slope,
                              int accum, float* __restrict__ out) {
    const float4* w4 = reinterpret_cast<const float4*>(ws);
    float4* o4 = reinterpret_cast<float4*>(out);
    for (int64_t i = (int64_t)blockIdx.x * blockDim.x + threadIdx.x; i < n4; i += (int64_t)gridDim.x * blockDim.x) {
        float4 s = w4[i];
        for (int k = 1; k < splitk; ++k) {
            float4 t = w4[i + k * stride4];
            s.x += t.x; s.y += t.y; s.z += t.z; s.w += t.w;
        }
        if (accum) {
            float4 t = o4[i];
            s.x += t.x; s.y += t.y; s.z += t.z; s.w += t.w;
        }
        s.x = s.x >= 0.f ? s.x : s.x * slope; s.y = s.y >= 0.f ? s.y : s.y * slope;
        s.z = s.z >= 0.f ? s.z : s.z * slope; s.w = s.w >= 0.f ? s.w : s.w * slope;
        o4[i] = s;
    }
}

__host__ __device__ inline int splitk_cgb(int CG) { return (CG & 63) == 0 ? 64 : ((CG & 31) == 0 ? 32 : 16); }

__global__ void __launch_bounds__(256) splitk_reduce_rows(const float* __restrict__ ws, int splitk, int64_t stride4,
                                                          int nvox, int Cout, int vpb, int nrows, float slope, int accum,
                                                          float* __restrict__ out, double* __restrict__ rsum,
                                                          double* __restrict__ rsq, float* __restrict__ rmn,
                                                          float* __restrict__ rmx) {
    __shared__ float4 lsh[4][256];
    const int CG = Cout >> 2;
    const int CGB = splitk_cgb(CG);
    const int NV = 256 / CGB;
    const int tid = threadIdx.x;
    const int cgl = tid % CGB, vl = tid / CGB;
    const int c4 = blockIdx.y * CGB + cgl;
    const int smp = blockIdx.z, rb = blockIdx.x;
    const int v0 = rb * vpb, v1 = min(nvox, v0 + vpb);
    const float4* w4 = reinterpret_cast<const float4*>(ws);
    float4* o4 = reinterpret_cast<float4*>(out);
    float4 fs = make_float4(0.f, 0.f, 0.f, 0.f), fq = fs;
    float4 mn = make_float4(INFINITY, INFINITY, INFINITY, INFINITY), mx = make_float4(-INFINITY, -INFINITY, -INFINITY, -INFINITY);
    for (int v = v0 + vl; v < v1; v += NV) {
        const int64_t i = ((int64_t)smp * nvox + v) * CG + c4;
        float4 a = w4[i];
        for (int k = 1; k < splitk; ++k) {
            const float4 t = w4[i + k * stride4];
            a.x += t.x; a.y += t.y; a.z += t.z; a.w += t.w;
        }
        if (accum) {
            const float4 t = o4[i];
            a.x += t.x; a.y += t.y; a.z += t.z; a.w += t.w;
        }
        a.x = a.x >= 0.f ? a.x : a.x * slope; a.y = a.y >= 0.f ? a.y : a.y * slope;
        a.z = a.z >= 0.f ? a.z : a.z * slope; a.w = a.w >= 0.f ? a.w : a.w * slope;
        o4[i] = a;
        fs.x += a.x; fs.y += a.y; fs.z += a.z; fs.w += a.w;
        fq.x = fmaf(a.x, a.x, fq.x); fq.y = fmaf(a.y, a.y, fq.y); fq.z = fmaf(a.z, a.z, fq.z); fq.w = fmaf(a.w, a.w, fq.w);
        mn.x = fminf(mn.x, a.x); mn.y = fminf(mn.y, a.y); mn.z = fminf(mn.z, a.z); mn.w = fminf(mn.w, a.w);
        mx.x = fmaxf(mx.x, a.x); mx.y = fmaxf(mx.y, a.y); mx.z = fmaxf(mx.z, a.z); mx.w = fmaxf(mx.w, a.w);
    }
    lsh[0][tid] = fs; lsh[1][tid] = fq; lsh[2][tid] = mn; lsh[3][tid] = mx;
    __syncthreads();
    if (vl == 0) {
        double S[4] = {0.0, 0.0, 0.0, 0.0}, Q[4] = {0.0, 0.0, 0.0, 0.0};
        float MN[4] = {INFINITY, INFINITY, INFINITY, INFINITY}, MX[4] = {-INFINITY, -INFINITY, -INFINITY, -INFINITY};
        for (int j = 0; j < NV; ++j) {
            const float4 a = lsh[0][j * CGB + cgl], b = lsh[1][j * CGB + cgl], c = lsh[2][j * CGB + cgl], d = lsh[3][j * CGB + cgl];
            S[0] += (double)a.x; S[1] += (double)a.y; S[2] += (double)a.z; S[3] += (double)a.w;
            Q[0] += (double)b.x; Q[1] += (double)b.y; Q[2] += (double)b.z; Q[3] += (double)b.w;
            MN[0] = fminf(MN[0], c.x); MN[1] = fminf(MN[1], c.y); MN[2] = fminf(MN[2], c.z); MN[3] = fminf(MN[3], c.w);
            MX[0] = fmaxf(MX[0], d.x); MX[1] = fmaxf(MX[1], d.y); MX[2] = fmaxf(MX[2], d.z); MX[3] = fmaxf(MX[3], d.w);
        }
        const size_t o = ((size_t)smp * nrows + rb) * Cout + (size_t)c4 * 4;
#pragma unroll
        for (int k = 0; k < 4; ++k) { rsum[o + k] = S[k]; rsq[o + k] = Q[k]; rmn[o + k] = MN[k]; rmx[o + k] = MX[k]; }
    }
}

static int splitk_rows_vpb(int64_t nvox, int Cout) {
    const int CG = Cout / 4, CGB = splitk_cgb(CG), NV = 256 / CGB;
    int64_t vpb = std::max<int64_t>((int64_t)NV * 4, bfm_cdiv64(nvox, 128));
    vpb = bfm_cdiv64(vpb, NV) * NV;
    return (int)std::min<int64_t>(vpb, 0x7fffffff);
}

constexpr int PK_ROW = KC * 27 + 1;
__global__ void __launch_bounds__(256) pack_mfma_tiled(const float* __restrict__ w, int Cin, int Cout, int wexp,
                                                       uint4* __restrict__ out) {
    extern __shared__ float pk_lds[];
    const int KCN = Cin / KC;
    const int nb = blockIdx.x & 1;
    const int kc = (blockIdx.x >> 1) % KCN, ntile = (blockIdx.x >> 1) / KCN;
    const float s = ldexpf(1.0f, wexp);
    const float* src0 = w + ((int64_t)(ntile * 64 + nb * 32) * Cin + kc * KC) * 27;
    bfm_stage_rows<32, KC * 27, PK_ROW, 256>(src0, (int64_t)Cin * 27, pk_lds, s,
                                             ((reinterpret_cast<uintptr_t>(w) & 15) == 0) && (Cin & 3) == 0);
    __syncthreads();
    uint4* dst = out + (int64_t)(blockIdx.x >> 1) * (27 * 2 * 2 * 64);
    const int lane = threadIdx.x & 63, wave = threadIdx.x >> 6;
    for (int tap = wave; tap < 27; tap += 4) {
        const float* src = pk_lds + (lane & 31) * PK_ROW + ((lane >> 5) * 8) * 27 + tap;
        half8 vh, vl;
#pragma unroll
        for (int j = 0; j < 8; ++j) {
            const float x = src[j * 27];
            const _Float16 hh = (_Float16)x;
            vh[j] = hh;
            vl[j] = (_Float16)(x - (float)hh);
        }
        dst[((tap * 2 + nb) * 2 + 0) * 64 + lane] = *reinterpret_cast<uint4*>(&vh);
        dst[((tap * 2 + nb) * 2 + 1) * 64 + lane] = *reinterpret_cast<uint4*>(&vl);
    }
}

__global__ void pack_mfma(const float* __restrict__ w, int Cin, int Cout, int wexp, uint4* __restrict__ out) {
    const int KCN = Cin / KC;
    const int64_t n = (int64_t)(Cout / 64) * KCN * 27 * 2 * 2 * 64;
    const float s = ldexpf(1.0f, wexp);
    for (int64_t i = (int64_t)blockIdx.x * blockDim.x + threadIdx.x; i < n; i += (int64_t)gridDim.x * blockDim.x) {
        int lane = (int)(i & 63);
        int64_t r = i >> 6;
        int hl = (int)(r & 1); r >>= 1;
        int nb = (int)(r & 1); r >>= 1;
        int tap = (int)(r % 27); r /= 27;
        int kc = (int)(r % KCN);
        int ntile = (int)(r / KCN);
        int co = ntile * 64 + nb * 32 + (lane & 31);
        int ci0 = kc * KC + (lane >> 5) * 8;
        half8 v;
#pragma unroll
        for (int j = 0; j < 8; ++j) {
            float x = w[((int64_t)co * Cin + ci0 + j) * 27 + tap] * s;
            _Float16 hh = (_Float16)x;
            v[j] = hl ? (_Float16)(x - (float)hh) : hh;
        }
        out[i] = *reinterpret_cast<uint4*>(&v);
    }
}

constexpr int nslot_for(int WN) { return WN == 1 ? 3 : 2; }
constexpr int ring_bytes(int WN) { return nslot_for(WN) * 12 * WN * 1024; }

struct HostPlan {
    int WM, WN, TD, TH, TW, splitk;
    int ver;
};

constexpr int LDS_LIMIT_WS = 160 * 1024;
int ws_smem(int npl, int plane_stride, int WN) { return 2 * (2 * npl * plane_stride) + 3 * 12 * WN * 1024; }

constexpr int LDS_LIMIT = 80 * 1024;

int plane_stride_for(int nvox) { return ((nvox * 16 + 63) / 64) * 64 + 32; }
int plane_stride16_for(int nvox) { return ((nvox * 16 + 127) / 128) * 128; }
constexpr int ring16_bytes(int WN) { return WN == 1 ? 2 * 2 * 8 * 1024 : 3 * 1 * 16 * 1024; }

bool is_pow2(int v) { return v > 0 && (v & (v - 1)) == 0; }
int ilog2(int v) { int s = 0; while ((1 << s) < v) ++s; return s; }

HostPlan choose_plan(int Cin, int Cout, int D, int H, int W) {
    HostPlan hp{};
    if (Cout % 128 == 0) { hp.WM = 2; hp.WN = 2; } else { hp.WM = 4; hp.WN = 1; }
    const int rows = hp.WM * 64;
    double best = 1e300;
    for (int tw = 1; tw <= std::min(W, 32); ++tw)
        for (int th = 1; th <= std::min(H, rows / tw); ++th) {
            int td = std::min(D, rows / (tw * th));
            if (td < 1) continue;
            int nvox = (td + 2) * (th + 2) * (tw + 2);
            if (4 * plane_stride_for(nvox) + ring_bytes(hp.WN) > LDS_LIMIT) continue;
            if (nvox * 4 > 12 * 64 * hp.WM * hp.WN) continue;
            double tiles = (double)bfm_cdiv(D, td) * bfm_cdiv(H, th) * bfm_cdiv(W, tw);
            double conflict = (tw % 16 == 0) ? 1.0 : 1.25;
            double cost = tiles * (rows * 27.0 + nvox * 4.0 * conflict);
            if (cost < best) { best = cost; hp.TD = td; hp.TH = th; hp.TW = tw; }
        }
    const int KCN = Cin / KC;
    int nMt = bfm_cdiv(D, hp.TD) * bfm_cdiv(H, hp.TH) * bfm_cdiv(W, hp.TW);
    int wgs = nMt * (Cout / (64 * hp.WN));
    hp.splitk = 1;
    if (wgs < 256 && KCN >= 8) {
        int want = bfm_cdiv(512, wgs);
        int maxs = KCN / 4;
        int s = std::min(want, maxs);
        if (s > 1) {
            int per = bfm_cdiv(KCN, s);
            hp.splitk = bfm_cdiv(KCN, per);
        }
    }
    hp.ver = (KCN >= 8 && hp.splitk == 1) ? 1 : 0;
    if (const char* e = getenv("BFM_CONV_VER")) hp.ver = atoi(e);
    return hp;
}

void launch16(const ConvParams& p, int passes, bool wm4, dim3 grid, size_t smem, hipStream_t st) {
    if (wm4) bfm_launch_by_passes(passes, conv_mfma16<4, 1, 3, 2, 2>, conv_mfma16<4, 1, 1, 2, 2>, grid, dim3(256), smem, st, p);
    else bfm_launch_by_passes(passes, conv_mfma16<2, 2, 3, 1, 3>, conv_mfma16<2, 2, 1, 1, 3>, grid, dim3(256), smem, st, p);
}

template <int WM, int WN>
int launch_ws(const ConvParams& p, int passes, dim3 grid, size_t smem, hipStream_t st) {
    static bool attr = false;
    if (const int rc = bfm_raise_lds_limit(attr, {bfm_kernel(&conv_mfma_ws<WM, WN, 3>), bfm_kernel(&conv_mfma_ws<WM, WN, 1>)},
                                           LDS_LIMIT_WS))
        return rc;
    bfm_launch_by_passes(passes, conv_mfma_ws<WM, WN, 3>, conv_mfma_ws<WM, WN, 1>, grid, dim3(512), smem, st, p);
    return BFM_OK;
}

template <int WM, int WN>
void launch(const ConvParams& p, int passes, dim3 grid, size_t smem, hipStream_t st) {
    bfm_launch_by_passes(passes, conv_mfma<WM, WN, 3, nslot_for(WN)>, conv_mfma<WM, WN, 1, nslot_for(WN)>, grid,
                         dim3(64 * WM * WN), smem, st, p);
}

}

extern "C" size_t bfm_pack_conv_weights_mfma_bytes(int Cin, int Cout) {
    if (Cin % KC || Cout % 64) return 0;
    return (size_t)(Cout / 64) * (Cin / KC) * 27 * 2 * 2 * 64 * 16;
}

extern "C" int bfm_pack_conv_weights_mfma(const float* w, int Cin, int Cout, float wmax_abs_host, void* wpacked,
                                          int* wexp_host, bfm_stream_t stream) {
    if (!w || !wpacked || !wexp_host || Cin <= 0 || Cout <= 0) return BFM_E_ARG;
    if (Cin % KC || Cout % 64) return BFM_E_SHAPE;
    int wexp = 0;
    if (wmax_abs_host > 0.f && wmax_abs_host < INFINITY) {
        int ex;
        (void)frexpf(wmax_abs_host, &ex);
        wexp = 14 - ex;
        wexp = wexp > 60 ? 60 : (wexp < -60 ? -60 : wexp);
    }
    *wexp_host = wexp;
    const int64_t nblk = (int64_t)(Cout / 64) * (Cin / KC) * 2;
    const size_t smem = (size_t)32 * PK_ROW * sizeof(float);
    static bool attr = false;
    if (const int rc = bfm_raise_lds_limit(attr, {bfm_kernel(&pack_mfma_tiled)}, (int)smem)) return rc;
    if (nblk <= 0x7fffffff) {
        hipLaunchKernelGGL(pack_mfma_tiled, dim3((unsigned)nblk), dim3(256), smem, bfm_s(stream), w, Cin, Cout, wexp,
                           reinterpret_cast<uint4*>(wpacked));
    } else {
        int64_t n = (nblk / 2) * 27 * 2 * 2 * 64;
        int nb = (int)std::min<int64_t>(4096, bfm_cdiv64(n, 256));
        hipLaunchKernelGGL(pack_mfma, dim3(nb), dim3(256), 0, bfm_s(stream), w, Cin, Cout, wexp,
                           reinterpret_cast<uint4*>(wpacked));
    }
    return bfm_launch_status();
}

extern "C" size_t bfm_pack_conv_weights_mfma16_bytes(int Cin, int Cout) {
    if (Cin % KC || Cout % 64) return 0;
    return (size_t)(Cout / 64) * (Cin / KC) * 14 * 4 * 2 * 64 * 16;
}

extern "C" int bfm_pack_conv_weights_mfma16(const float* w, int Cin, int Cout, float wmax_abs_host, void* wpacked,
                                            int* wexp_host, bfm_stream_t stream) {
    if (!w || !wpacked || !wexp_host || Cin <= 0 || Cout <= 0) return BFM_E_ARG;
    if (Cin % KC || Cout % 64) return BFM_E_SHAPE;
    int wexp = 0;
    if (wmax_abs_host > 0.f && wmax_abs_host < INFINITY) {
        int ex;
        (void)frexpf(wmax_abs_host, &ex);
        wexp = 14 - ex;
        wexp = wexp > 60 ? 60 : (wexp < -60 ? -60 : wexp);
    }
    *wexp_host = wexp;
    const int64_t nblk = (int64_t)(Cout / 64) * (Cin / KC) * 2;
    if (nblk <= 0x7fffffff) {
        const size_t smem = (size_t)32 * PK16_ROW * sizeof(float);
        static bool attr = false;
        if (const int rc = bfm_raise_lds_limit(attr, {bfm_kernel(&pack_mfma16_tiled)}, (int)smem)) return rc;
        hipLaunchKernelGGL(pack_mfma16_tiled, dim3((unsigned)nblk), dim3(256), smem, bfm_s(stream), w, Cin, Cout, wexp,
                           reinterpret_cast<uint4*>(wpacked));
        return bfm_launch_status();
    }
    int64_t n = (int64_t)(Cout / 64) * (Cin / KC) * 14 * 4 * 2 * 64;
    int nb = (int)std::min<int64_t>(4096, bfm_cdiv64(n, 256));
    hipLaunchKernelGGL(pack_mfma16, dim3(nb), dim3(256), 0, bfm_s(stream), w, Cin, Cout, wexp,
                       reinterpret_cast<uint4*>(wpacked));
    return bfm_launch_status();
}

extern "C" int bfm_conv3x3x3_mfma_plan(int Cin, int Cout, int D, int H, int W, int* cfg) {
    if (!cfg || Cin <= 0 || Cout <= 0 || D <= 0 || H <= 0 || W <= 0) return BFM_E_ARG;
    if (Cin % KC || Cout % 64) return BFM_E_SHAPE;
    HostPlan hp = choose_plan(Cin, Cout, D, H, W);
    if (hp.TD == 0) return BFM_E_SHAPE;
    cfg[0] = hp.WM; cfg[1] = hp.WN; cfg[2] = hp.TD; cfg[3] = hp.TH; cfg[4] = hp.TW; cfg[5] = hp.splitk;
    cfg[6] = hp.ver; cfg[7] = 0;
    return BFM_OK;
}

extern "C" size_t bfm_conv3x3x3_mfma_workspace(int Cin, int Cout, int D, int H, int W, int splitk) {
    (void)Cin;
    if (splitk <= 1) return 0;
    return (size_t)splitk * D * H * W * Cout * sizeof(float);
}

extern "C" int bfm_conv3x3x3_mfma_rows(int Cin, int Cout, int D, int H, int W, const int* cfg) {
    if (!cfg || Cin <= 0 || Cout <= 0 || D <= 0 || H <= 0 || W <= 0) return 0;
    if (cfg[6] >= 3 || cfg[6] < 0) return 0;
    int splitk = cfg[5] < 1 ? 1 : cfg[5];
    const int KCN = Cin / KC;
    if (splitk > KCN) splitk = KCN;
    if (splitk > 1 && bfm_cdiv(KCN, bfm_cdiv(KCN, splitk)) > 1) {
        if (Cout % 64) return 0;
        const int64_t nvox = (int64_t)D * H * W;
        return (int)bfm_cdiv64(nvox, splitk_rows_vpb(nvox, Cout));
    }
    if (cfg[6] == 1) return 0;
    if (cfg[2] < 1 || cfg[3] < 1 || cfg[4] < 1) return 0;
    return bfm_cdiv(D, cfg[2]) * bfm_cdiv(H, cfg[3]) * bfm_cdiv(W, cfg[4]);
}

extern "C" int bfm_conv3x3x3_mfma_ex(const float* A, int CA, const float* B, int CB, int D, int H, int W,
                                     const bfm_upsample_t* up, const float* scale, const float* shift,
                                     const float* bound, int G, const void* wpacked, int wexp, int Cout, float slope,
                                     int passes, const int* cfg, float* out, void* workspace, size_t workspace_bytes,
                                     void* moment_rows, bfm_stream_t stream);

extern "C" int bfm_conv3x3x3_mfma(const float* A, int CA, const float* B, int CB, int D, int H, int W,
                                  const bfm_upsample_t* up, const float* scale, const float* shift,
                                  const float* bound, int G, const void* wpacked, int wexp, int Cout, float slope,
                                  int passes, const int* cfg, float* out, void* workspace, size_t workspace_bytes,
                                  bfm_stream_t stream) {
    return bfm_conv3x3x3_mfma_ex(A, CA, B, CB, D, H, W, up, scale, shift, bound, G, wpacked, wexp, Cout, slope, passes,
                                 cfg, out, workspace, workspace_bytes, nullptr, stream);
}

static int conv_mfma_launch(const float* A, int CA, const float* B, int CB, int S, int D, int H, int W,
                            const bfm_upsample_t* up, const float* scale, const float* shift, const float* bound, int G,
                            const void* wpacked, int wexp, int Cout, float slope, int passes, const int* cfg, float* out,
                            void* workspace, size_t workspace_bytes, void* moment_rows, int affine_stride, bfm_stream_t stream);

extern "C" int bfm_conv3x3x3_mfma_ex(const float* A, int CA, const float* B, int CB, int D, int H, int W,
                                     const bfm_upsample_t* up, const float* scale, const float* shift,
                                     const float* bound, int G, const void* wpacked, int wexp, int Cout, float slope,
                                     int passes, const int* cfg, float* out, void* workspace, size_t workspace_bytes,
                                     void* moment_rows, bfm_stream_t stream) {
    return conv_mfma_launch(A, CA, B, CB, 1, D, H, W, up, scale, shift, bound, G, wpacked, wexp, Cout, slope, passes, cfg,
                            out, workspace, workspace_bytes, moment_rows, 0, stream);
}

#ifdef BFM_STAMPS
extern "C" int bfm_debug_stamps(long long* host_out) {
    return (int)hipMemcpyFromSymbol(host_out, HIP_SYMBOL(g_stamps), sizeof(long long) * 4096);
}
#endif

extern "C" size_t bfm_conv3x3x3_mfma_batch_workspace(int Cin, int Cout, int S, int D, int H, int W, int splitk) {
    return (size_t)(S < 1 ? 1 : S) * bfm_conv3x3x3_mfma_workspace(Cin, Cout, D, H, W, splitk);
}

extern "C" int bfm_conv3x3x3_mfma_batch(const float* A, int CA, const float* B, int CB, int S, int D, int H, int W,
                                        const bfm_upsample_t* up, const float* scale, const float* shift,
                                        const float* bound, int G, const void* wpacked, int wexp, int Cout, float slope,
                                        int passes, const int* cfg, float* out, void* workspace, size_t workspace_bytes,
                                        void* moment_rows, int affine_stride, bfm_stream_t stream) {
    if (S < 1 || !cfg) return BFM_E_ARG;
    if (affine_stride != 0 && (affine_stride < CA + CB || (affine_stride & 3))) return BFM_E_ARG;
    if (cfg[6] != 0 && cfg[6] != 2) return BFM_E_SHAPE;
    return conv_mfma_launch(A, CA, B, CB, S, D, H, W, up, scale, shift, bound, G, wpacked, wexp, Cout, slope, passes, cfg,
                            out, workspace, workspace_bytes, moment_rows, affine_stride, stream);
}

static int conv_mfma_launch(const float* A, int CA, const float* B, int CB, int S, int D, int H, int W,
                            const bfm_upsample_t* up, const float* scale, const float* shift, const float* bound, int G,
                            const void* wpacked, int wexp, int Cout, float slope, int passes, const int* cfg, float* out,
                            void* workspace, size_t workspace_bytes, void* moment_rows, int affine_stride,
                            bfm_stream_t stream) {
    if (!A || CA <= 0 || D <= 0 || H <= 0 || W <= 0 || !scale || !shift || !bound || G <= 0 || !wpacked || !out)
        return BFM_E_ARG;
    if (CB < 0 || (CB > 0 && (!B || !up || !up->mapD || !up->mapH || !up->mapW || up->d <= 0 || up->h <= 0 ||
                              up->w <= 0)))
        return BFM_E_ARG;
    if (CA % KC || CB % KC || Cout % 64) return BFM_E_SHAPE;
    if (passes != 1 && passes != 3) return BFM_E_ARG;
    if ((reinterpret_cast<uintptr_t>(A) & 15) || (CB > 0 && (reinterpret_cast<uintptr_t>(B) & 15)) ||
        (reinterpret_cast<uintptr_t>(scale) & 15) || (reinterpret_cast<uintptr_t>(shift) & 15) ||
        (reinterpret_cast<uintptr_t>(wpacked) & 15) || (reinterpret_cast<uintptr_t>(out) & 15))
        return BFM_E_ARG;
    const int Cin = CA + CB;
    HostPlan hp;
    if (cfg) {
        hp = HostPlan{cfg[0], cfg[1], cfg[2], cfg[3], cfg[4], cfg[5], cfg[6]};
    } else {
        hp = choose_plan(Cin, Cout, D, H, W);
    }
    const bool wg_ok = (hp.WM == 4 && hp.WN == 1) || (hp.WM == 2 && hp.WN == 2);
    if (!wg_ok || hp.TD < 1 || hp.TH < 1 || hp.TW < 1 || hp.TD * hp.TH * hp.TW > hp.WM * 64) return BFM_E_SHAPE;
    if (Cout % (64 * hp.WN)) return BFM_E_SHAPE;
    if (hp.TD + 2 > 1023 || hp.TH + 2 > 1023 || hp.TW + 2 > 1023) return BFM_E_SHAPE;

    ConvParams p{};
    p.A = A; p.B = B; p.CA = CA; p.CB = CB; p.D = D; p.H = H; p.W = W;
    p.up = make_upview(up);
    p.scale = scale; p.shift = shift; p.bound = bound; p.G = G;
    p.wp = reinterpret_cast<const uint4*>(wpacked);
    p.wexp = wexp; p.Cout = Cout; p.slope = slope;
    p.accum = (cfg && (cfg[7] & 1)) ? 1 : 0;
    p.TD = hp.TD; p.TH = hp.TH; p.TW = hp.TW; p.HT = hp.TH + 2; p.WT = hp.TW + 2;
    const int nTz = bfm_cdiv(D, hp.TD);
    p.nTy = bfm_cdiv(H, hp.TH); p.nTx = bfm_cdiv(W, hp.TW);
    p.nMtS = nTz * p.nTy * p.nTx;
    p.S = S;
    p.saff = affine_stride > 0 ? affine_stride : CA + CB;
    p.nMt = S * p.nMtS;
    p.NT = Cout / (64 * hp.WN);
    p.KCN = Cin / KC;
    p.splitk = hp.splitk < 1 ? 1 : hp.splitk;
    if (p.splitk > p.KCN) p.splitk = p.KCN;
    p.kc_per_split = bfm_cdiv(p.KCN, p.splitk);
    p.splitk = bfm_cdiv(p.KCN, p.kc_per_split);
    p.nvox_lds = (hp.TD + 2) * p.HT * p.WT;
    p.plane_stride = hp.ver == 2 ? plane_stride16_for(p.nvox_lds) : plane_stride_for(p.nvox_lds);
    p.tw_shift = is_pow2(hp.TW) ? ilog2(hp.TW) : -1;
    p.thw_shift = is_pow2(hp.TH * hp.TW) ? ilog2(hp.TH * hp.TW) : -1;
    const int npl = passes == 3 ? 2 : 1;
    const size_t smem = hp.ver == 1 ? (size_t)ws_smem(npl, p.plane_stride, hp.WN)
                        : hp.ver == 2 ? (size_t)2 * npl * p.plane_stride + ring16_bytes(hp.WN)
                                      : (size_t)2 * npl * p.plane_stride + ring_bytes(hp.WN);
    if (smem > (size_t)(hp.ver == 1 ? LDS_LIMIT_WS : LDS_LIMIT)) return BFM_E_SHAPE;
    if (hp.ver < 0 || hp.ver > 2) return BFM_E_ARG;
    if (p.nvox_lds * 4 > 12 * 64 * hp.WM * hp.WN) return BFM_E_SHAPE;
    const int64_t nvox = (int64_t)D * H * W;
    p.sA = nvox * CA;
    p.sB = CB > 0 ? (int64_t)up->d * up->h * up->w * CB : 0;
    p.sO = nvox * Cout;
    p.split_stride = (int64_t)S * nvox * Cout;
    if (p.splitk > 1) {
        if (!workspace || workspace_bytes < (size_t)p.splitk * S * nvox * Cout * sizeof(float)) return BFM_E_WORKSPACE;
        if (reinterpret_cast<uintptr_t>(workspace) & 15) return BFM_E_ARG;
        p.out = static_cast<float*>(workspace);
    } else {
        p.out = out;
    }
    if (moment_rows && p.splitk > 1) {
        if (reinterpret_cast<uintptr_t>(moment_rows) & 7) return BFM_E_ARG;
    } else if (moment_rows) {
        if (hp.ver == 1) return BFM_E_SHAPE;
        MomentRows rows;
        if (!rows.carve(moment_rows, (size_t)p.nMt * Cout)) return BFM_E_ARG;
        rows.into(p);
    }
#ifdef BFM_MFMA_ABLATE
    if (const char* e = getenv("BFM_MFMA_ABL")) p.abl = atoi(e);
#endif
    if ((int64_t)hp.TD * H * W * Cout > 0x7fffffffLL) return BFM_E_SHAPE;
    if ((int64_t)p.nMt * p.NT > 0x7fffffff) return BFM_E_SHAPE;
    if (nvox * CA > 0x7fffffffLL || (CB > 0 && (int64_t)up->d * up->h * up->w * CB > 0x7fffffffLL))
        return BFM_E_SHAPE;
    unsigned gx = (unsigned)(p.nMt * p.NT);
    if (hp.ver == 1) {
        const int cap = 256;
        if ((int)gx > cap) gx = (unsigned)cap;
    }
    dim3 grid(gx, (unsigned)p.splitk);
    hipStream_t st = bfm_s(stream);
    if (hp.ver == 2) {
        launch16(p, passes, hp.WM == 4, grid, smem, st);
    } else if (hp.ver == 1) {
        if (const int rc = hp.WM == 4 ? launch_ws<4, 1>(p, passes, grid, smem, st) : launch_ws<2, 2>(p, passes, grid, smem, st))
            return rc;
    } else {
        if (hp.WM == 4) launch<4, 1>(p, passes, grid, smem, st);
        else launch<2, 2>(p, passes, grid, smem, st);
    }
    int rc = bfm_launch_status();
    if (rc != BFM_OK) return rc;
    if (p.splitk > 1 && moment_rows) {
        if (nvox > 0x7fffffffLL || S > 65535) return BFM_E_SHAPE;
        const int vpb = splitk_rows_vpb(nvox, Cout);
        const int nrows = (int)bfm_cdiv64(nvox, vpb);
        const int CG = Cout / 4, CGB = splitk_cgb(CG);
        MomentRows rows;
        (void)rows.carve(moment_rows, (size_t)S * nrows * Cout);
        hipLaunchKernelGGL(splitk_reduce_rows, dim3(nrows, CG / CGB, S), dim3(256), 0, st,
                           static_cast<const float*>(workspace), p.splitk, p.split_stride / 4, (int)nvox, Cout, vpb, nrows,
                           slope, p.accum, out, rows.rsum, rows.rsq, rows.rmn, rows.rmx);
        rc = bfm_launch_status();
    } else if (p.splitk > 1) {
        int64_t n4 = (int64_t)S * nvox * Cout / 4;
        int nb = (int)std::min<int64_t>(2048, bfm_cdiv64(n4, 256));
        hipLaunchKernelGGL(splitk_reduce, dim3(nb), dim3(256), 0, st, static_cast<const float*>(workspace), p.splitk,
                           n4, p.split_stride / 4, slope, p.accum, out);
        rc = bfm_launch_status();
    }
    return rc;
}
```

### include/brainfm_hip.h

```cpp
#ifndef BRAINFM_HIP_H
#define BRAINFM_HIP_H

#include <stddef.h>
#include <stdint.h>

#ifdef __cplusplus
extern "C" {
#endif

typedef void* bfm_stream_t;

#define BFM_OK 0
#define BFM_E_ARG (-1)
#define BFM_E_SHAPE (-2)
#define BFM_E_WORKSPACE (-3)
#define BFM_E_LAUNCH (-4)

typedef struct {
    int d, h, w;
    const int32_t* mapD; const int32_t* mapH; const int32_t* mapW;
    const int32_t* repD; const int32_t* repH; const int32_t* repW;
} bfm_upsample_t;

const char* bfm_version(void);

size_t bfm_gn_stats_workspace(int CA, int CB, int D, int H, int W, const bfm_upsample_t* up);
int bfm_gn_stats(const float* A, int CA, const float* B, int CB, int D, int H, int W,
                 const bfm_upsample_t* up, const float* gamma, const float* beta, int G, float eps,
                 float* scale, float* shift, float* bound, void* workspace, size_t workspace_bytes,
                 bfm_stream_t stream);
int bfm_gn_stats_train(const float* A, int CA, const float* B, int CB, int D, int H, int W, const bfm_upsample_t* up,
                       const float* gamma, const float* beta, int G, float eps, float* scale, float* shift,
                       float* bound, float* mean_out, float* rstd_out, void* workspace, size_t workspace_bytes,
                       bfm_stream_t stream);

int bfm_pack_conv_weights_direct(const float* w_oidhw, int Cin, int Cout, float* wpacked, bfm_stream_t stream);
size_t bfm_pack_conv_weights_mfma_bytes(int Cin, int Cout);
int bfm_pack_conv_weights_mfma(const float* w_oidhw, int Cin, int Cout, float wmax_abs_host, void* wpacked,
                               int* wexp_host, bfm_stream_t stream);

size_t bfm_pack_conv_weights_mfma16_bytes(int Cin, int Cout);
int bfm_pack_conv_weights_mfma16(const float* w_oidhw, int Cin, int Cout, float wmax_abs_host, void* wpacked,
                                 int* wexp_host, bfm_stream_t stream);

int bfm_conv3x3x3_direct(const float* A, int CA, const float* B, int CB, int D, int H, int W,
                         const bfm_upsample_t* up, const float* scale, const float* shift,
                         const float* wpacked, int Cout, float slope, float* out, bfm_stream_t stream);


size_t bfm_pack_conv_weights_wino_bytes(int Cin, int Cout, int passes);
int bfm_pack_conv_weights_wino(const float* w_oidhw, int Cin, int Cout, float wmax_abs_host, int passes, void* wpacked,
                               int* wexp_host, bfm_stream_t stream);
int bfm_conv3x3x3_wino_rows(int D, int H, int W, int passes);
int bfm_conv3x3x3_wino_ex(const float* A, int CA, int D, int H, int W, const float* scale, const float* shift,
                          const float* bound, int G, const void* wpacked, int wexp, int Cout, float slope, int passes,
                          int flags, float* out, void* moment_rows , bfm_stream_t stream);

size_t bfm_uniform_boxes_bytes(int D, int H, int W, int passes);
int bfm_uniform_boxes(const float* image, int D, int H, int W, int radius, int passes, unsigned char* flags,
                      bfm_stream_t stream);
int bfm_uniform_boxes_level(const float* image, int D, int H, int W, int level, int radius, int passes, unsigned char* flags,
                            bfm_stream_t stream);
size_t bfm_conv3x3x3_wino_uniform_scratch(int Cout);
int bfm_conv3x3x3_wino_uniform(const float* A, int CA, int D, int H, int W, const float* scale, const float* shift,
                               const float* bound, int G, const void* wpacked, int wexp, int Cout, float slope, int passes,
                               int flags, float* out, void* moment_rows, const unsigned char* uniform_flags, void* scratch,
                               bfm_stream_t stream);
int bfm_conv3x3x3_wino_pool_ok(int D, int H, int W, int passes);
int bfm_conv3x3x3_wino_pool(const float* A, int CA, int D, int H, int W, const float* scale, const float* shift,
                            const float* bound, int G, const void* wpacked, int wexp, int Cout, float slope, int passes,
                            int flags, float* out, void* moment_rows, float* pooled, void* pooled_rows ,
                            bfm_stream_t stream);
int bfm_conv3x3x3_wino_uniform_pool(const float* A, int CA, int D, int H, int W, const float* scale, const float* shift,
                                    const float* bound, int G, const void* wpacked, int wexp, int Cout, float slope,
                                    int passes, int flags, float* out, void* moment_rows,
                                    const unsigned char* uniform_flags, void* scratch, float* pooled,
                                    void* pooled_rows , bfm_stream_t stream);
int bfm_conv3x3x3_wino_box(int D, int H, int W, int passes, int* box );
size_t bfm_conv3x3x3_wino_masked_workspace(int D, int H, int W, int passes);
int bfm_conv3x3x3_wino_masked(const float* A, int CA, int D, int H, int W, const float* scale, const float* shift,
                              const float* bound, int G, const void* wpacked, int wexp, int Cout, float slope, int passes,
                              int flags, float* out, const float* mask_image, void* workspace, size_t workspace_bytes,
                              bfm_stream_t stream);

size_t bfm_moment_rows_bytes(int nrows, int C);
int bfm_conv3x3x3_mfma_rows(int Cin, int Cout, int D, int H, int W, const int* cfg);
int bfm_conv3x3x3_mfma_ex(const float* A, int CA, const float* B, int CB, int D, int H, int W,
                          const bfm_upsample_t* up, const float* scale, const float* shift, const float* bound,
                          int G, const void* wpacked, int wexp, int Cout, float slope, int passes, const int* cfg,
                          float* out, void* workspace, size_t workspace_bytes, void* moment_rows ,
                          bfm_stream_t stream);
size_t bfm_conv3x3x3_mfma_batch_workspace(int Cin, int Cout, int S, int D, int H, int W, int splitk);
int bfm_conv3x3x3_mfma_batch(const float* A, int CA, const float* B, int CB, int S, int D, int H, int W,
                             const bfm_upsample_t* up, const float* scale, const float* shift, const float* bound, int G,
                             const void* wpacked, int wexp, int Cout, float slope, int passes, const int* cfg, float* out,
                             void* workspace, size_t workspace_bytes, void* moment_rows, int affine_stride,
                             bfm_stream_t stream);
size_t bfm_gn_stats_batch_workspace(int CA, int CB, int S, int D, int H, int W, const bfm_upsample_t* up);
int bfm_gn_stats_batch(const float* A, int CA, const float* B, int CB, int S, int D, int H, int W,
                       const bfm_upsample_t* up, const float* gamma, const float* beta, int G, float eps, float* scale,
                       float* shift, float* bound, void* workspace, size_t workspace_bytes, bfm_stream_t stream);
int bfm_gn_stats_rows_batch(const void* rowsA, int nrowsA_per_sample, int CA, const void* rowsB, int nrowsB_per_sample,
                            int CB, double weightB, int64_t nvox, int S, const float* gamma, const float* beta, int G,
                            float eps, float* scale, float* shift, float* bound, bfm_stream_t stream);

int bfm_maxpool2_rows(int C, int D, int H, int W);
int bfm_maxpool2_ex(const float* in, int C, int D, int H, int W, float* out, void* moment_rows ,
                    bfm_stream_t stream);
int bfm_maxpool2_batch_rows(int C, int D, int H, int W);
int bfm_maxpool2_batch(const float* in, int C, int S, int D, int H, int W, float* out, void* moment_rows ,
                       bfm_stream_t stream);
int bfm_conv3x3x3_stem_rows(int D, int H, int W);
int bfm_conv3x3x3_stem_ex(const float* A, int D, int H, int W, const float* scale, const float* shift,
                          const float* bound, const float* wpacked_direct, int Cout, float slope, float* out,
                          void* moment_rows , bfm_stream_t stream);
int bfm_conv3x3x3_stem_mc_ex(const float* A, int Cin, int D, int H, int W, const float* scale, const float* shift,
                             const float* bound, const float* wpacked_direct, int Cout, float slope, float* out,
                             void* moment_rows , bfm_stream_t stream);
size_t bfm_gn_stats_rows_workspace(int nrowsA, int CA, int nrowsB, int CB);
#define BFM_GN_TICKETS 16
int bfm_gn_stats_rows(const void* rowsA, int nrowsA, int CA, const void* rowsB, int nrowsB, int CB, double weightB,
                      int64_t nvox, const float* gamma, const float* beta, int G, float eps, float* scale,
                      float* shift, float* bound, void* workspace, size_t workspace_bytes, void* ticket,
                      bfm_stream_t stream);
int bfm_gn_stats_rows_train(const void* rowsA, int nrowsA, int CA, const void* rowsB, int nrowsB, int CB, double weightB,
                            int64_t nvox, const float* gamma, const float* beta, int G, float eps, float* scale,
                            float* shift, float* bound, float* mean_out, float* rstd_out, void* workspace,
                            size_t workspace_bytes, void* ticket, bfm_stream_t stream);

int bfm_gn_stats_rows_sliced(const void* rowsA, int totalA, int firstA, int nrowsA, int CA, const void* rowsB, int totalB,
                             int firstB, int nrowsB, int CB, double weightB, int64_t nvox, const float* gamma,
                             const float* beta, int G, float eps, float* scale, float* shift, float* bound,
                             void* workspace, size_t workspace_bytes, void* ticket, bfm_stream_t stream);

size_t bfm_pack_conv_weights_wino4_bytes(int Cin, int Cout, int passes);
int bfm_pack_conv_weights_wino4(const float* w_oidhw, int Cin, int Cout, float wmax_abs_host, int passes, void* wpacked,
                                int* wexp_host, bfm_stream_t stream);
int bfm_conv3x3x3_wino4_rows(int D, int H, int W, int passes);
int bfm_conv3x3x3_wino4_box(int D, int H, int W, int passes, int* box );
int bfm_conv3x3x3_wino4(const float* A, int CA, int D, int H, int W, const float* scale, const float* shift,
                        const float* bound, int G, const void* wpacked, int wexp, int Cout, float slope, int passes,
                        int flags, float* out, void* moment_rows , bfm_stream_t stream);
int bfm_conv3x3x3_wino4_batch(const float* A, int CA, int S, int D, int H, int W, const float* scale, const float* shift,
                              const float* bound, int G, const void* wpacked, int wexp, int Cout, float slope, int passes,
                              int flags, float* out, void* moment_rows, int affine_stride, bfm_stream_t stream);
size_t bfm_conv3x3x3_wino4_masked_workspace(int D, int H, int W, int passes);
size_t bfm_conv3x3x3_wino4_uniform_scratch(int Cout);
int bfm_conv3x3x3_wino4_uniform(const float* A, int CA, int D, int H, int W, const float* scale, const float* shift,
                                const float* bound, int G, const void* wpacked, int wexp, int Cout, float slope, int passes,
                                int flags, float* out, void* moment_rows, const unsigned char* uniform_flags, void* scratch,
                                bfm_stream_t stream);
int bfm_conv3x3x3_wino4_masked(const float* A, int CA, int D, int H, int W, const float* scale, const float* shift,
                               const float* bound, int G, const void* wpacked, int wexp, int Cout, float slope, int passes,
                               int flags, float* out, const float* mask_image, void* workspace, size_t workspace_bytes,
                               bfm_stream_t stream);

size_t bfm_conv3x3x3_mfma_workspace(int Cin, int Cout, int D, int H, int W, int splitk);
int bfm_conv3x3x3_mfma_plan(int Cin, int Cout, int D, int H, int W, int* cfg_out );

size_t bfm_pack_conv_weights_upfold_bytes(int CB, int Cout, int passes);
int bfm_pack_conv_weights_upfold(const float* w_oidhw , int CA, int CB, int Cout,
                                 float wmax_abs_host, int passes, void* wpacked, int* wexp_host, bfm_stream_t stream);
int bfm_conv3x3x3_upfold(const float* B, int CB, int d, int h, int w, const float* scale_b, const float* shift_b,
                         const float* bound, int G, const void* wpacked, int wexp, int Cout, int passes, float* out,
                         bfm_stream_t stream);
size_t bfm_conv3x3x3_upfold_workspace(int CB, int d, int h, int w, int Cout);
int bfm_conv3x3x3_upfold_ex(const float* B, int CB, int d, int h, int w, const float* scale_b, const float* shift_b,
                            const float* bound, int G, const void* wpacked, int wexp, int Cout, int passes, float* out,
                            void* workspace, size_t workspace_bytes, bfm_stream_t stream);
size_t bfm_conv3x3x3_upfold_batch_workspace(int CB, int S, int d, int h, int w, int Cout);
int bfm_conv3x3x3_upfold_batch(const float* B, int CB, int S, int d, int h, int w, const float* scale_b,
                               const float* shift_b, const float* bound, int G, const void* wpacked, int wexp, int Cout,
                               int passes, float* out, void* workspace, size_t workspace_bytes, int affine_stride,
                               bfm_stream_t stream);

int bfm_conv3x3x3_mfma(const float* A, int CA, const float* B, int CB, int D, int H, int W,
                       const bfm_upsample_t* up, const float* scale, const float* shift, const float* bound,
                       int G, const void* wpacked, int wexp, int Cout, float slope, int passes,
                       const int* cfg , float* out, void* workspace,
                       size_t workspace_bytes, bfm_stream_t stream);

int bfm_maxpool2(const float* in, int C, int D, int H, int W, float* out, bfm_stream_t stream);

enum {
    BFM_ROLE_PLAIN = 0,
    BFM_ROLE_CT = 1,
    BFM_ROLE_BIAS_LOG = 2,
    BFM_ROLE_SEG = 3,
    BFM_ROLE_DIST = 4,
    BFM_ROLE_SR = 5,
    BFM_ROLE_PATHOL = 6
};
typedef struct {
    int n_out;
    int c_feat;
    const float* head_w;
    const float* head_b;
    const int32_t* roles;
    const int32_t* out_slot;
    int seg_first, n_seg;
    const int32_t* seg_lut;
    int n_dist;
    int dist_first;
    float max_dist;
    int unit_feat;
    int slot_high_res;
    int slot_fake_cortical;
    int n_maps;
    float head_wmax;
    int skip_zero_input;
} bfm_tail_desc_t;

int bfm_tail_heads(const float* feat, const float* input , int64_t nvox,
                   const bfm_tail_desc_t* desc, float* feat_norm ,
                   float* const* maps ,
                   float* seg_prob , int64_t* label ,
                   float* raw_out ,
                   bfm_stream_t stream);
int bfm_tail_heads_rows(const float* feat, const float* input , int64_t nvox,
                        const bfm_tail_desc_t* desc, float* feat_norm , float* maps_rows, int64_t row_stride,
                        float* seg_prob , int64_t* label , int flags, bfm_stream_t stream);

int bfm_stitch_accumulate(const float* tile, const int64_t* tile_label, const float* tile_input,
                          int td, int th, int tw, float* full, int D, int H, int W,
                          int z0, int y0, int x0, bfm_stream_t stream);
int bfm_stitch_accumulate_multi(const float* maps, int64_t map_stride, const int32_t* sel, int K,
                                const int64_t* tile_label, const float* tile_input, int td, int th, int tw, float* full,
                                int D, int H, int W, int z0, int y0, int x0, bfm_stream_t stream);
int bfm_tile_count_add(float* cnt, int D, int H, int W, int z0, int z1, int y0, int y1, int x0, int x1,
                       bfm_stream_t stream);
int bfm_pack_tile_multi(const float* maps, int64_t map_stride, const int32_t* sel, int K, const int64_t* tile_label,
                        const float* tile_input, int64_t n, float* out, bfm_stream_t stream);
int bfm_divide_by_count_multi(float* full, const float* cnt, int64_t vol, int K, bfm_stream_t stream);
int bfm_stitch_gather_multi(const int64_t* tiles, int T, int K, float* full, int D, int H, int W, bfm_stream_t stream);

int bfm_tile_mask_blocks(int64_t tile_voxels);
int bfm_tile_mask_index(const float* volume, int D, int H, int W, const int64_t* tiles, int T, int total_blocks,
                        int32_t* pos, int32_t* nnz, int32_t* block_ws, bfm_stream_t stream);
int bfm_pack_tile_compact(const float* maps, int64_t map_stride, const int32_t* sel, int K, const int64_t* tile_label,
                          const float* tile_input, int64_t n, const int32_t* pos, int64_t row_stride, float* out,
                          bfm_stream_t stream);
int bfm_stitch_gather_compact(const int64_t* tiles, int T, int K, const float* volume, float* full, int D, int H, int W,
                              bfm_stream_t stream);

enum {
    BFM_EW_EXP = 0, BFM_EW_AFFINE = 1 , BFM_EW_CLAMP = 2 , BFM_EW_CLAMP_MIN = 3,
    BFM_EW_GAMMA = 4 , BFM_EW_SIGMOID = 5,
    BFM_EW_DIV = 6 , BFM_EW_NONZERO = 7 , BFM_EW_SUB_DIV = 8 ,
    BFM_EW_GE = 9 ,
    BFM_EW_NAN_TO_NUM = 10
};
enum {
    BFM_EW_ADD = 0, BFM_EW_MUL = 1, BFM_EW_MUL_EXP = 2 ,
    BFM_EW_AXPY_CLAMP0 = 3 , BFM_EW_AXPY = 4, BFM_EW_DIV2 = 5,
    BFM_EW_ZERO_WHERE_ZERO = 6
};
int bfm_ew_unary(int op, const float* in, int64_t in_stride, float* out, int64_t out_stride, int64_t n,
                 float a, float b, bfm_stream_t stream);
int bfm_ew_binary(int op, const float* x, int64_t x_stride, const float* y, int64_t y_stride ,
                  float* out, int64_t out_stride, int64_t n, float a, bfm_stream_t stream);
int bfm_absmax_f32(const float* x, int64_t rows, int64_t len, int64_t row_stride, float* out_zeroed, bfm_stream_t stream);
int bfm_softmax_cl(const float* x, int64_t x_row_stride, int C, float* y, int64_t y_row_stride, int64_t n,
                   bfm_stream_t stream);
int bfm_argmax_lut_cl(const float* p, int64_t row_stride, int C, const int32_t* lut, int64_t* out, int64_t n,
                      bfm_stream_t stream);
int bfm_fake_cortical(const float* dist, int64_t row_stride, int n_dist, float* out, int64_t n,
                      bfm_stream_t stream);
int bfm_mask_concat2(const float* x, const float* p, int64_t n, float* out, bfm_stream_t stream);
int bfm_condition_input(const float* x, const float* p, int mode, int D, int H, int W, float* out, float* masked,
                        float* flipped, bfm_stream_t stream);

int bfm_interp3d_linear(const float* X, int nx, int ny, int nz, int C, const float* II, const float* JJ,
                        const float* KK, int64_t n, float default_value, float* out, bfm_stream_t stream);
int bfm_interp3d_nearest(const void* X, int nx, int ny, int nz, int C, const float* II, const float* JJ,
                         const float* KK, int64_t n, void* out, bfm_stream_t stream);
int bfm_deformed_atlas(const float* mask, const float* regx, const float* regy, const float* regz, const float* atlas,
                       int nx, int ny, int nz, const float* A_host, int64_t n, float* out, bfm_stream_t stream);
int bfm_deformed_atlas_tile(const float* tile_in, const float* regx, const float* regy, const float* regz,
                            const float* atlas, int nx, int ny, int nz, const float* A_host, int64_t n, float* out,
                            bfm_stream_t stream);
typedef struct { const int32_t* f; const int32_t* c; const float* wf; const float* wc; } bfm_zoom_axis_t;
int bfm_zoom_linear(const float* X, int nx, int ny, int nz, int C, const bfm_zoom_axis_t* axes , int ox, int oy,
                    int oz, float* out, bfm_stream_t stream);
int bfm_conv1d_axis(const float* in, int nx, int ny, int nz, int axis, const float* kern, int klen, float* out,
                    bfm_stream_t stream);
int bfm_grid_push3d_linear(const float* inp, int Bi, int C, int ix, int iy, int iz, const float* grid, int Bg, int nx,
                           int ny, int nz, const int* bound, int extrapolate, float* out_zeroed, bfm_stream_t stream);
int bfm_grid_grad3d_linear(const float* inp, int Bi, int C, int nx, int ny, int nz, const float* grid, int Bg, int ox,
                           int oy, int oz, const int* bound, int extrapolate, float* out, bfm_stream_t stream);

int bfm_crop3d(const float* vol, int D, int H, int W, int z0, int y0, int x0, int d, int h, int w, float* out,
               bfm_stream_t stream);

int bfm_permute_flip3d(const float* in, int nx, int ny, int nz, const int* perm ,
                       const int* flip , float* out, bfm_stream_t stream);
int bfm_bbox_nonzero(const float* in, int nx, int ny, int nz, float tol, int32_t* box ,
                     bfm_stream_t stream);
int bfm_mean_lastdim(const float* in, int64_t n, int c, float* out, bfm_stream_t stream);

int bfm_bspline3_prefilter_axis(float* vol, int nx, int ny, int nz, int axis, int bound, float pole, float gain,
                                const float* init_w, float pole_last, float init_scale, float final_scale,
                                bfm_stream_t stream);
int bfm_bspline3_resample_axis(const float* in, int nx, int ny, int nz, int axis, const float* coord, int n_out,
                               int bound, float* out, bfm_stream_t stream);

int bfm_grid_pull3d_linear(const float* inp, int Bi, int C, int nx, int ny, int nz, const float* grid, int Bg, int ox,
                           int oy, int oz, const int* bound, int extrapolate, float* out, bfm_stream_t stream);
size_t bfm_deform_grid_workspace(int sx, int sy, int sz);
int bfm_deform_grid(const float* F, int sx, int sy, int sz, const float* A_host , const float* c2_host ,
                    const int* shp_host , float* xx, float* yy, float* zz, float* minmax ,
                    void* workspace, size_t workspace_bytes, bfm_stream_t stream);
#define BFM_CLASS_STATS_BLOCKS 1024
int bfm_label_class_stats(const float* G, const float* syn, int64_t n, float* cerebral, double* stats ,
                          double* partials, bfm_stream_t stream);
int bfm_label_gauss(const float* G, const float* mus, const float* sigmas, const float* randn, int64_t n, int ntab,
                    float* out, bfm_stream_t stream);
int bfm_onehot_lut(const int32_t* S, const int32_t* lut, int nlut, int n_labels, int64_t n, float* out,
                   bfm_stream_t stream);

int bfm_perlin3d(const double* grad, int sx, int sy, int sz, int rx, int ry, int rz, double* out, bfm_stream_t stream);
int bfm_radix_hist_f64(const double* x, int64_t n, uint64_t prefix, int shift, uint32_t* hist65536, bfm_stream_t stream);
int bfm_threshold_mask_f64(const double* x, int64_t n, double thr, double* masked, double* mask, bfm_stream_t stream);
int bfm_curl3d(const double* a, const double* b, const double* c, int sx, int sy, int sz, float mult, float* Vx,
               float* Vy, float* Vz, bfm_stream_t stream);
int bfm_advect_upwind_rhs(const void* C, int c_is_f64, const float* Vx, const float* Vy, const float* Vz, int sx,
                          int sy, int sz, int neumann_bc, float* out, bfm_stream_t stream);
typedef struct { const float* k[7]; float coef[7]; int nk; } bfm_kset_t;
int bfm_rk_combine(const void* y0 , int is_f64, const bfm_kset_t* ks, void* out, int64_t n,
                   bfm_stream_t stream);
size_t bfm_reduce_workspace(void);
int bfm_rk_error_sumsq(const bfm_kset_t* ks, const void* y0, const void* y1, int is_f64, double atol, double rtol,
                       int64_t n, double* out, void* workspace, size_t workspace_bytes, bfm_stream_t stream);
int bfm_scaled_sumsq(const void* a, const void* b , int ab_is_f64, const void* y0, int y_is_f64,
                     double atol, double rtol, int64_t n, double* out, void* workspace, size_t workspace_bytes,
                     bfm_stream_t stream);
int bfm_dopri5_dense_eval(const void* y0, const void* y1, int is_f64, const bfm_kset_t* mid, double dt, double x,
                          void* out, int64_t n, bfm_stream_t stream);
int bfm_reduce_f32(int op, const float* x, const float* y, int64_t n, double* out, void* workspace,
                   size_t workspace_bytes, bfm_stream_t stream);
int bfm_reduce_f64(int op, const double* x, const double* y, int64_t n, double* out, void* workspace,
                   size_t workspace_bytes, bfm_stream_t stream);


int bfm_randn_philox(float* out, int64_t n, uint64_t seed, uint64_t offset, float scale, bfm_stream_t stream);

size_t bfm_deform_zoom_workspace(void);
int bfm_deform_zoom_minmax(const float* Fsmall, int fnx, int fny, int fnz, const bfm_zoom_axis_t* ax, int photo_zero_y,
                           int sx, int sy, int sz, const float* A_host, const float* c2_host, const int* shp_host,
                           float* minmax6, void* workspace, size_t workspace_bytes, bfm_stream_t stream);
int bfm_deform_zoom_write(const float* Fsmall, int fnx, int fny, int fnz, const bfm_zoom_axis_t* ax, int photo_zero_y,
                          int sx, int sy, int sz, const float* A_host, const float* c2_host, const int* shp_host,
                          const float* lo_host , float* xx, float* yy, float* zz, float* F_out ,
                          bfm_stream_t stream);

size_t bfm_svf_integrate_workspace(int sx, int sy, int sz);
int bfm_svf_integrate(const float* F, int sx, int sy, int sz, int n_steps, float* F_out, float* Fneg_out, void* workspace,
                      size_t workspace_bytes, bfm_stream_t stream);
#define BFM_VERTEX_SETS_MAX 4
typedef struct {
    float* V;
    int64_t n;
} bfm_vertex_set_t;
int bfm_deform_vertices(const float* Fneg, int sx, int sy, int sz, const bfm_vertex_set_t* sets, int n_sets,
                        const float* Ainv_host, const float* c2_host, int flip, int size0, bfm_stream_t stream);

#define BFM_GATHER_MAX_JOBS 12
typedef struct {
    const float* src; float* out;
    float mean, scale; int pre; int default_max;
    float post_div; int clamp; float clamp_lo, clamp_hi; float sign; int want_minmax;
} bfm_gather_job_t;
size_t bfm_gather_targets_workspace(void);
int bfm_gather_targets(const bfm_gather_job_t* jobs, int njobs, int nx, int ny, int nz, const int* box6_host,
                       const float* II, const float* JJ, const float* KK, int sx, int sy, int sz, int flip0,
                       double* scalars, void* workspace, size_t workspace_bytes, bfm_stream_t stream);
int bfm_minmax_normalise(float* x, int64_t n, const double* minmax_dev, bfm_stream_t stream);
int bfm_gather_onehot(const int32_t* S, int nx, int ny, int nz, const int* box6_host, const float* II, const float* JJ,
                      const float* KK, int sx, int sy, int sz, int flip0, const int32_t* lut, int nlut, int n_labels,
                      const int32_t* vflip , float* out, bfm_stream_t stream);
int bfm_gather_onehot_rows(const int32_t* S, int nx, int ny, int nz, const int* box6_host, const float* II, const float* JJ,
                      const float* KK, int sx, int sy, int sz, int flip0, const int32_t* lut, int nlut, int n_labels,
                      const int32_t* vflip , float* out, bfm_stream_t stream);

size_t bfm_percentile_workspace(void);
int bfm_percentile_f64(const double* x, int64_t n, int64_t k_lo, int need_next, double t, double* out3, void* workspace,
                       size_t workspace_bytes, bfm_stream_t stream);
size_t bfm_shape_workspace(void);
int bfm_shape_threshold_f64(const double* noise, int64_t n, const double* thr_dev, double* masked, double* mask,
                            double* max_out, void* workspace, size_t workspace_bytes, bfm_stream_t stream);
int bfm_shape_binarize(const void* p, int is_f64, int64_t n, const double* max_dev, double thres, void* P,
                       double* sum_out, void* workspace, size_t workspace_bytes, bfm_stream_t stream);
int bfm_pathology_mask(void* P, void* Pprob, int is_f64, const float* cerebral, int64_t n, double* sum_out,
                       void* workspace, size_t workspace_bytes, bfm_stream_t stream);
size_t bfm_pathology_encode_workspace(void);
int bfm_pathology_encode_dev(const float* I, const void* P, const void* Pprob, int is_f64, const float* randn,
                             const float* u4_host, int direction, const double* class_stats_dev, int64_t n, float* out,
                             double* dotsum_out, void* workspace, size_t workspace_bytes, bfm_stream_t stream);
int bfm_interp3d_linear_axes(const float* X, int nx, int ny, int nz, const float* ax, const float* ay, const float* az,
                             int ox, int oy, int oz, float default_value, float* out, bfm_stream_t stream);
int bfm_sample_finalize(const float* I, const float* high_res, int sx, int sy, int sz, const double* max_dev, int flip0,
                        float* input_out, float* residual_out, bfm_stream_t stream);

typedef struct {
    void* y[2]; float* f[2]; float* k[5];
    const float *Vx, *Vy, *Vz;
    int sx, sy, sz, neumann_bc, is_f64;
    double atol, rtol, tol_min_dt, dt_max, safety, ifactor, dfactor;
    const double* t_out ; int nt; void* sol ;
    void* state; void* workspace;
} bfm_dopri5_advect_t;
size_t bfm_dopri5_advect_state_bytes(void);
size_t bfm_dopri5_advect_workspace(int sx, int sy, int sz);
int bfm_dopri5_advect_init(const bfm_dopri5_advect_t* d, double t0, double dt0, bfm_stream_t stream);
int bfm_dopri5_advect_steps(const bfm_dopri5_advect_t* d, int nsteps, bfm_stream_t stream);

int bfm_lrelu_bwd(const float* dY, const float* Y, int64_t n, float slope, float* dP, bfm_stream_t stream);
int bfm_lrelu_bwd_ex(const float* dY, const float* Y, int64_t n, float slope, float* dP, float* absmax,
                     bfm_stream_t stream);
size_t bfm_conv3x3x3_wgrad_workspace(int Cin, int Cout, int D, int H, int W);
size_t bfm_stem_mc_bwd_workspace(int Cin, int Cout, int D, int H, int W);
int bfm_stem_mc_bwd(const float* dP, int Cout, const float* x, int Cin, int D, int H, int W, const float* w_raw,
                    const float* scale, const float* shift, const float* mean, const float* rstd,
                    float* dW , float* dgamma , float* dbeta , void* workspace,
                    size_t workspace_bytes, bfm_stream_t stream);
int bfm_conv3x3x3_wgrad(const float* dP, int Cout, const float* A, int CA, const float* B, int CB, int D, int H, int W,
                        const bfm_upsample_t* up, const float* scale, const float* shift, float* dW ,
                        void* workspace, size_t workspace_bytes, bfm_stream_t stream);
int bfm_conv3x3x3_wgrad_ex(const float* dP, int Cout, const float* A, int CA, const float* B, int CB, int D, int H, int W,
                           const bfm_upsample_t* up, const float* scale, const float* shift, const float* dp_bound,
                           const float* x_bound, int G, int passes, float* dW, void* workspace, size_t workspace_bytes,
                           bfm_stream_t stream);
size_t bfm_gn_bwd_workspace(int C, int D, int H, int W);
int bfm_gn_bwd(const float* dXn, const float* A, int CA, const float* B, int CB, int D, int H, int W,
               const bfm_upsample_t* up, const int32_t* startD, const int32_t* startH, const int32_t* startW,
               const float* mean, const float* rstd, const float* gamma, int G, float* dA, float* dB, float* dgamma,
               float* dbeta, void* workspace, size_t workspace_bytes, bfm_stream_t stream);
int bfm_maxpool2_bwd(const float* in, const float* dOut, int C, int D, int H, int W, float* dIn, bfm_stream_t stream);
int bfm_transpose_mirror_weights(const float* w_oidhw, int Cout, int Cin, int CinPad, float* out, bfm_stream_t stream);

size_t bfm_loss_workspace(int ns);
int bfm_loss_l1(const float* raw, int n_out, int co, const float* target, const float* weight, const float* mask_mul,
                int64_t nvox, float clampv, int l2 , float coef,
                float* dRaw, double* loss_out, void* workspace, size_t workspace_bytes, bfm_stream_t stream);
size_t bfm_loss_l1_multi_workspace(void);
int bfm_loss_l1_multi(const float* raw, int n_out, int64_t nvox, int n, const int32_t* cols, const int32_t* l2,
                      const float* clampv, const float* coef, const float* const* targets, const float* const* weights,
                      const float* const* masks, float* dRaw, double* loss_out, void* workspace, size_t workspace_bytes,
                      bfm_stream_t stream);
int bfm_loss_grad_l1(const float* raw, int n_out, int co, const float* target, const float* weight, int D, int H, int W,
                     float coef, float* dRaw, double* loss_out, void* workspace, size_t workspace_bytes,
                     bfm_stream_t stream);
int bfm_loss_grad_l1_multi(const float* raw, int n_out, int n, const int32_t* cols, const float* coef,
                           const float* const* targets, const float* const* weights, int D, int H, int W, float* dRaw,
                           double* loss_out, void* workspace, size_t workspace_bytes, bfm_stream_t stream);
int bfm_loss_seg(const float* raw, int n_out, int c0, int ns, const float* target, const float* wce, const float* wdice,
                 int64_t nvox, float coef_ce, float coef_dice, float* P, float* dRaw, double* loss_out ,
                 void* workspace, size_t workspace_bytes, bfm_stream_t stream);
size_t bfm_loss_pathol_workspace(void);
int bfm_loss_pathol(const float* raw, int64_t col_offset, int64_t voxel_stride, const float* target, int64_t nvox,
                    float coef_ce, float coef_dice, float* dRaw, double* loss_ce, double* loss_dice, void* workspace,
                    size_t workspace_bytes, bfm_stream_t stream);
size_t bfm_loss_reg_workspace(int nch, int D, int H, int W);
int bfm_loss_reg_smooth(const float* raw, int64_t col_offset, int64_t chan_stride, int64_t voxel_stride, int nch, int D, int H,
                        int W, float coef, float* dRaw, double* loss_out, void* workspace, size_t workspace_bytes,
                        bfm_stream_t stream);
int bfm_loss_reg_hessian(const float* raw, int64_t col_offset, int64_t chan_stride, int64_t voxel_stride, int nch, int D, int H,
                         int W, float coef, float* dRaw, double* loss_out, void* workspace, size_t workspace_bytes,
                         bfm_stream_t stream);
size_t bfm_loss_contrastive_workspace(void);
int bfm_loss_contrastive(const float* featP, const float* featQ, int C, int64_t nvox, int n_norm, float eps, float alpha,
                         float beta, float gamma, float coef, float* dP, float* dQ, float* p_out, float* q_out,
                         double* loss_out, void* workspace, size_t workspace_bytes, bfm_stream_t stream);
size_t bfm_head_bwd_workspace(int n_out, int C, int64_t nvox);
int bfm_head_bwd(const float* dRaw, const float* Fn, const float* head_w, int n_out, int C, int64_t nvox, float* dW,
                 float* db, float* dFn, void* workspace, size_t workspace_bytes, bfm_stream_t stream);
int bfm_tail_raw_rows(const float* feat, int64_t nvox, const bfm_tail_desc_t* desc, float* feat_norm, float* raw_rows,
                      int64_t row_stride, bfm_stream_t stream);
int bfm_loss_l1_multi_rows(const float* raw_rows, int64_t row_stride, int n_out, int64_t nvox, int n, const int32_t* cols,
                           const int32_t* l2, const float* clampv, const float* coef, const float* const* targets,
                           const float* const* weights, const float* const* masks, float* dRaw_rows, double* loss_out,
                           void* workspace, size_t workspace_bytes, bfm_stream_t stream);
int bfm_loss_grad_l1_multi_rows(const float* raw_rows, int64_t row_stride, int n_out, int n, const int32_t* cols,
                                const float* coef, const float* const* targets, const float* const* weights, int D, int H,
                                int W, float* dRaw_rows, double* loss_out, void* workspace, size_t workspace_bytes,
                                bfm_stream_t stream);
int bfm_loss_seg_rows(const float* raw_rows, int64_t row_stride, int n_out, int c0, int ns, const float* target,
                      const float* wce, const float* wdice, int64_t nvox, float coef_ce, float coef_dice, float* P,
                      float* dRaw_rows, double* loss_out , void* workspace, size_t workspace_bytes,
                      bfm_stream_t stream);
int bfm_head_bwd_rows(const float* dRaw_rows, int64_t row_stride, const float* Fn, const float* head_w, int n_out, int C,
                      int64_t nvox, float* dW, float* db, float* dFn, void* workspace, size_t workspace_bytes,
                      bfm_stream_t stream);
int bfm_normalize_bwd(const float* feat, const float* dFn, int C, int64_t nvox, float eps, float* dfeat,
                      bfm_stream_t stream);
typedef struct bfm_adam_tensor {
    float* p; const float* g; float* m; float* v;
    int64_t n;
    float grad_scale, bias1, bias2_sqrt;
    int32_t first_chunk;
    int64_t reserved;
} bfm_adam_tensor_t;
int bfm_grad_sumsq_multi(const bfm_adam_tensor_t* tensors, int ntensors, const int32_t* chunk_tensor, int nchunks,
                         int64_t chunk_elems, double* sums_out, int32_t* nonfinite, void* workspace, size_t workspace_bytes,
                         bfm_stream_t stream);
int bfm_adamw_step_multi(const bfm_adam_tensor_t* tensors, int ntensors, const int32_t* chunk_tensor, int nchunks,
                         int64_t chunk_elems, float lr, float beta1, float beta2, float eps, float weight_decay,
                         bfm_stream_t stream);
int bfm_adamw_step(float* p, const float* g, float* m, float* v, int64_t n, float lr, float beta1, float beta2,
                   float eps, float weight_decay, int step, float grad_scale, bfm_stream_t stream);
int bfm_grad_sumsq(const float* g, int64_t n, double* out, int32_t* nonfinite, void* workspace, size_t workspace_bytes,
                   bfm_stream_t stream);

typedef struct bfm_age_params {
    const float *c1w, *c1b;
    const float *c2w, *c2b;
    const float *l1w, *l1b;
    const float *l2w, *l2b;
    const float *l3w, *l3b;
} bfm_age_params_t;
typedef struct bfm_age_grads {
    float *c1w, *c1b, *c2w, *c2b, *l1w, *l1b, *l2w, *l2b, *l3w, *l3b;
} bfm_age_grads_t;
int bfm_maxpool4(const float* in, int C, int D, int H, int W, float* out, uint8_t* arg, bfm_stream_t stream);
int bfm_maxpool4_bwd(const float* g, const uint8_t* arg, int C, int D, int H, int W, float* dst, int accumulate,
                     bfm_stream_t stream);
int bfm_age_conv_fwd(const float* x, int Cin, int D, int H, int W, const float* w, const float* b, int Cout, float* y,
                     bfm_stream_t stream);
size_t bfm_age_conv_bwd_workspace(int Cin, int D, int H, int W, int Cout);
int bfm_age_conv_bwd(const float* x, int Cin, int D, int H, int W, const float* w, int Cout, const float* y, const float* dy,
                     float* dx, float* dw, float* db, void* workspace, size_t workspace_bytes, bfm_stream_t stream);
int bfm_age_mlp_fwd(const float* y2, int nv, const bfm_age_params_t* prm, int n_flat, float* h1, float* h2, float* out,
                    bfm_stream_t stream);
size_t bfm_age_mlp_bwd_workspace(void);
int bfm_age_mlp_bwd(const float* y2, int nv, const bfm_age_params_t* prm, int n_flat, const float* h1, const float* h2,
                    const float* p, const float* dp_in, double age, float coef, double* loss, const bfm_age_grads_t* grd,
                    float* dy2, void* workspace, size_t workspace_bytes, bfm_stream_t stream);

#ifdef __cplusplus
}
#endif
#endif
```

Before: 200.2 million voxels/s.

## Pack multiple small batched samples into one MFMA conv workgroup M-tile

Adds a packed mode to the batched MFMA 3D conv kernels. When each sample's volume is small enough (deep UNet levels), several samples share one workgroup's M rows. Each packed sample gets its own halo region in LDS, its own per-sample affine/exponent scaling, and per-sample moment rows computed from an LDS-staged output tile. This targets underfilled M tiles and wasted MFMA work at tiny spatial sizes, at the cost of more LDS, extra per-element affine lookups and a separate epilogue reduction. It is on by default and can be disabled with BFM_PACK_M=0.

```diff
diff --git a/brainfm_amd/_lib.py b/brainfm_amd/_lib.py
--- a/brainfm_amd/_lib.py
+++ b/brainfm_amd/_lib.py
@@ -105,6 +105,7 @@
     "bfm_conv3x3x3_mfma_ex": (_I, [_P, _I, _P, _I, _I, _I, _I, _UP, _P, _P, _P, _I, _P, _I, _I, _F, _I,
                                    C.POINTER(_I), _P, _P, _Z, _P, _P]),
     "bfm_conv3x3x3_mfma_batch_workspace": (_Z, [_I, _I, _I, _I, _I, _I, _I]),
+    "bfm_conv3x3x3_mfma_batch_pack": (_I, [_I, _I, _I, _I, _I, _I, C.POINTER(_I), _I, _I]),
     "bfm_conv3x3x3_mfma_batch": (_I, [_P, _I, _P, _I, _I, _I, _I, _I, _UP, _P, _P, _P, _I, _P, _I, _I, _F, _I,
                                       C.POINTER(_I), _P, _P, _Z, _P, _I, _P]),
     "bfm_gn_stats_batch_workspace": (_Z, [_I, _I, _I, _I, _I, _I, _UP]),
diff --git a/brainfm_amd/csrc/conv3d_mfma.hip b/brainfm_amd/csrc/conv3d_mfma.hip
--- a/brainfm_amd/csrc/conv3d_mfma.hip
+++ b/brainfm_amd/csrc/conv3d_mfma.hip
@@ -41,6 +41,9 @@
     double *rsum, *rsq;
     float *rmn, *rmx;
     int abl;
+    int P, pvox, phalo;
+    int pk_tail;
+    int oTH, oTW, oboxN;
 };
 
 
@@ -110,7 +113,87 @@
     return tab;
 }
 
-template <int WM, int WN, int NPASS, int NSLOT>
+
+__device__ __forceinline__ int aexp_of_bound(const float* pb, int G) {
+    float bmax = 0.f;
+    for (int g = 0; g < G; ++g) bmax = fmaxf(bmax, pb[g]);
+    int aexp = 0;
+    if (bmax > 0.f && bmax < INFINITY) {
+        int ex;
+        (void)frexpf(bmax, &ex);
+        aexp = 14 - ex;
+        aexp = aexp > 60 ? 60 : (aexp < -60 ? -60 : aexp);
+    }
+    return aexp;
+}
+
+template <int ROWS, int NTHR>
+__device__ __forceinline__ const int* build_row_table_pk(const ConvParams& p, unsigned char* lds, int tid, int nsub) {
+    int* tab = reinterpret_cast<int*>(lds);
+    const int* aex = reinterpret_cast<const int*>(lds + p.pk_tail);
+    for (int q = tid; q < ROWS; q += NTHR) {
+        const int sub = q / p.pvox;
+        int rel = -1, ae = 0;
+        if (sub < nsub) {
+            rel = sub * (int)p.sO + (q - sub * p.pvox) * p.Cout;
+            ae = aex[sub];
+        }
+        tab[q] = rel;
+        tab[ROWS + q] = ae;
+    }
+    return tab;
+}
+
+template <int WM, int WN, bool M16>
+__device__ __forceinline__ void store_moment_rows_pk(const ConvParams& p, unsigned char* lds, int tid, int smp0, int nsub,
+                                                     int nt) {
+    constexpr int ROWS = WM * 64, NTHR = 64 * WM * WN, NC = 64 * WN;
+    int* emu = reinterpret_cast<int*>(lds);
+    const float* tile = reinterpret_cast<const float*>(lds + ROWS * 8);
+    __syncthreads();
+    for (int q = tid; q < ROWS; q += NTHR) {
+        int e = -1;
+        if (q < p.oboxN) {
+            const int d = q / (p.oTH * p.oTW), rem = q - d * (p.oTH * p.oTW);
+            const int h = rem / p.oTW, w = rem - h * p.oTW;
+            if (d < p.D && h < p.H && w < p.W) e = (d * p.H + h) * p.W + w;
+        }
+        emu[q] = e;
+    }
+    __syncthreads();
+    for (int item = tid; item < nsub * NC; item += NTHR) {
+        const int sub = item / NC, c = item - sub * NC;
+        const float* col = tile + (size_t)sub * p.pvox * NC + c;
+        double S = 0.0, Q = 0.0;
+        float MN = INFINITY, MX = -INFINITY;
+        for (int m = 0; m < WM && m * 64 < p.oboxN; ++m) {
+            constexpr int NKG = M16 ? 4 : 2;
+            double ks[NKG], kq[NKG];
+#pragma unroll
+            for (int kg = 0; kg < NKG; ++kg) {
+                float fs = 0.f, fq = 0.f;
+                for (int a = 0; a < (M16 ? 4 : 8); ++a) {
+                    const int q0 = M16 ? m * 64 + a * 16 + kg * 4 : m * 64 + (a >> 2) * 32 + row_perm((a & 3) * 8 + kg * 4);
+#pragma unroll
+                    for (int j = 0; j < 4; ++j) {
+                        const int e = emu[q0 + j];
+                        if (e < 0) continue;
+                        const float r = col[(size_t)e * NC];
+                        fs += r; fq = fmaf(r, r, fq);
+                        MN = fminf(MN, r); MX = fmaxf(MX, r);
+                    }
+                }
+                ks[kg] = (double)fs; kq[kg] = (double)fq;
+            }
+            if constexpr (M16) { S += (ks[0] + ks[1]) + (ks[2] + ks[3]); Q += (kq[0] + kq[1]) + (kq[2] + kq[3]); }
+            else { S += ks[0] + ks[1]; Q += kq[0] + kq[1]; }
+        }
+        const size_t o = (size_t)(smp0 + sub) * p.Cout + nt * NC + c;
+        p.rsum[o] = S; p.rsq[o] = Q; p.rmn[o] = MN; p.rmx[o] = MX;
+    }
+}
+
+template <int WM, int WN, int NPASS, int NSLOT, bool PK = false>
 __global__ void __launch_bounds__(64 * WM * WN, 2) conv_mfma(const ConvParams p) {
     constexpr int NTHR = 64 * WM * WN;
     constexpr int NW = WM * WN;
@@ -135,7 +218,11 @@
         bid = (xcd < r ? xcd * (q + 1) : r * (q + 1) + (xcd - r) * q) + idx;
     }
     int mt, nt, smp = 0;
-    if (p.S > 1) {
+    if constexpr (PK) {
+        mt = bid % p.nMt;
+        nt = bid / p.nMt;
+        smp = mt * p.P;
+    } else if (p.S > 1) {
         smp = bid % p.S;
         const int t = bid / p.S;
         nt = t % p.NT;
@@ -144,7 +231,8 @@
         mt = bid / p.NT;
         nt = bid - mt * p.NT;
     }
-    const int mtl = mt - smp * p.nMtS;
+    const int mtl = PK ? 0 : mt - smp * p.nMtS;
+    const int nsub = PK ? min(p.P, p.S - smp) : 1;
     const float* const pA = p.A + smp * p.sA;
     const float* const pB = p.B + smp * p.sB;
     const float* const pscale = p.scale + smp * p.saff;
@@ -163,6 +251,12 @@
     const int z0 = tz * p.TD, y0 = ty * p.TH, x0 = tx * p.TW;
     const int boxN = p.TD * p.TH * p.TW;
 
+    int* const pk_aexp = reinterpret_cast<int*>(lds + p.pk_tail);
+    float* const pk_aff = reinterpret_cast<float*>(pk_aexp + ((p.P + 3) & ~3));
+    if constexpr (PK) {
+        if (tid < p.P) pk_aexp[tid] = tid < nsub ? aexp_of_bound(pbound + tid * p.G, p.G) : 0;
+        __syncthreads();
+    }
     float bmax = 0.f;
     for (int g = 0; g < p.G; ++g) bmax = fmaxf(bmax, pbound[g]);
     int aexp = 0;
@@ -179,9 +273,12 @@
 #pragma unroll
     for (int mb = 0; mb < 2; ++mb) {
         int q = wm * 64 + mb * 32 + row_perm(l32);
-        int d = 0, h = 0, w = 0;
-        if (q < boxN) box_coords(p, q, d, h, w);
-        int vox = (d * p.HT + h) * p.WT + w;
+        int d = 0, h = 0, w = 0, vbase = 0;
+        if constexpr (PK) {
+            const int sub = q / p.pvox;
+            if (sub < p.P) { box_coords(p, q - sub * p.pvox, d, h, w); vbase = sub * p.phalo; }
+        } else if (q < boxN) box_coords(p, q, d, h, w);
+        int vox = vbase + (d * p.HT + h) * p.WT + w;
         a_off[mb] = (khalf * NPL) * p.plane_stride + vox * 16;
     }
 
@@ -189,6 +286,7 @@
     const int n_el = p.nvox_lds * 4;
     const int q4 = tid & 3;
     int off[MAX_IT];
+    int ssubp[MAX_IT / 4] = {0, 0, 0};
     auto compute_offsets = [&](bool fromB) {
 #pragma unroll
         for (int it = 0; it < MAX_IT; ++it) {
@@ -196,15 +294,22 @@
             off[it] = -2;
             if (e < n_el) {
                 const int vox = e >> 2;
-                const int hz = vox / (p.HT * p.WT);
+                int hz = vox / (p.HT * p.WT);
                 const int rem = vox - hz * (p.HT * p.WT);
+                int sub = 0;
+                if constexpr (PK) {
+                    sub = hz / (p.D + 1);
+                    hz -= sub * (p.D + 1);
+                    ssubp[it >> 2] |= min(sub, nsub - 1) << ((it & 3) * 8);
+                }
                 const int hy = rem / p.WT;
                 const int hx = rem - hy * p.WT;
                 const int gz = z0 + hz - 1, gy = y0 + hy - 1, gx = x0 + hx - 1;
                 off[it] = -1;
-                if (gz >= 0 && gz < p.D && gy >= 0 && gy < p.H && gx >= 0 && gx < p.W) {
-                    if (fromB) off[it] = ((p.up.mapD[gz] * p.up.h + p.up.mapH[gy]) * p.up.w + p.up.mapW[gx]) * p.CB;
-                    else off[it] = ((gz * p.H + gy) * p.W + gx) * p.CA;
+                if (PK && sub >= nsub) {
+                } else if (gz >= 0 && gz < p.D && gy >= 0 && gy < p.H && gx >= 0 && gx < p.W) {
+                    if (!PK && fromB) off[it] = ((p.up.mapD[gz] * p.up.h + p.up.mapH[gy]) * p.up.w + p.up.mapW[gx]) * p.CB;
+                    else off[it] = (PK ? sub * (int)p.sA : 0) + ((gz * p.H + gy) * p.W + gx) * p.CA;
                 }
             }
         }
@@ -224,7 +329,8 @@
     const int ntw = nt * WN + wn;
     if (p.accum && p.splitk == 1) {
         const float inv_dq = ldexpf(1.0f, aexp + p.wexp);
-        const int* rowtab = build_row_table<WM * 64, NTHR>(p, lds, tid, z0, y0, x0, boxN);
+        const int* rowtab = PK ? build_row_table_pk<WM * 64, NTHR>(p, lds, tid, nsub)
+                               : build_row_table<WM * 64, NTHR>(p, lds, tid, z0, y0, x0, boxN);
         __syncthreads();
         const float* ib = pout + (((int64_t)z0 * p.H + y0) * p.W + x0) * p.Cout + ntw * 64 + l32;
 #pragma unroll
@@ -233,12 +339,18 @@
             for (int ig = 0; ig < 4; ++ig) {
                 const int4 r4 = *reinterpret_cast<const int4*>(rowtab + wm * 64 + mb * 32 + row_perm(ig * 8 + khalf * 4));
                 const int rel[4] = {r4.x, r4.y, r4.z, r4.w};
+                int ae[4] = {0, 0, 0, 0};
+                if constexpr (PK) {
+                    const int4 e4 = *reinterpret_cast<const int4*>(rowtab + WM * 64 + wm * 64 + mb * 32 + row_perm(ig * 8 + khalf * 4));
+                    ae[0] = e4.x; ae[1] = e4.y; ae[2] = e4.z; ae[3] = e4.w;
+                }
 #pragma unroll
                 for (int j = 0; j < 4; ++j) {
                     if (rel[j] < 0) continue;
                     const float* orow = ib + (unsigned)rel[j];
-#pragma unroll
-                    for (int nb = 0; nb < 2; ++nb) acc[mb][nb][ig * 4 + j] = orow[nb * 32] * inv_dq;
+                    const float idq = PK ? ldexpf(1.0f, ae[j] + p.wexp) : inv_dq;
+#pragma unroll
+                    for (int nb = 0; nb < 2; ++nb) acc[mb][nb][ig * 4 + j] = orow[nb * 32] * idq;
                 }
             }
         }
@@ -281,6 +393,13 @@
         const float4 sh4 = *reinterpret_cast<const float4*>(pshift + c0 + q4 * 4);
         const float sc[4] = {sc4.x * a_scale, sc4.y * a_scale, sc4.z * a_scale, sc4.w * a_scale};
         const float sh[4] = {sh4.x * a_scale, sh4.y * a_scale, sh4.z * a_scale, sh4.w * a_scale};
+        if constexpr (PK) {
+            for (int i = tid; i < p.P * 32; i += NTHR) {
+                const int sb = min(i >> 5, nsub - 1), c = i & 15;
+                const float* row = ((i & 16) ? pshift : pscale) + sb * p.saff + c0;
+                pk_aff[i] = row[c] * ldexpf(1.0f, pk_aexp[sb]);
+            }
+        }
 
         STAMP((kc - kc_begin) * 8 + 0);
         __syncthreads();
@@ -299,10 +418,20 @@
                 if (off[it0 + u] != -2) {
                     const bool ok = off[it0 + u] >= 0;
                     float y[4] = {v[u].x, v[u].y, v[u].z, v[u].w};
+                    float scu[4], shu[4];
+                    if constexpr (PK) {
+                        const float* af = pk_aff + ((ssubp[(it0 + u) >> 2] >> (((it0 + u) & 3) * 8)) & 255) * 32 + q4 * 4;
+                        const float4 a4 = *reinterpret_cast<const float4*>(af), b4 = *reinterpret_cast<const float4*>(af + 16);
+                        scu[0] = a4.x; scu[1] = a4.y; scu[2] = a4.z; scu[3] = a4.w;
+                        shu[0] = b4.x; shu[1] = b4.y; shu[2] = b4.z; shu[3] = b4.w;
+                    } else {
+#pragma unroll
+                        for (int i = 0; i < 4; ++i) { scu[i] = sc[i]; shu[i] = sh[i]; }
+                    }
                     half4 hi, lo;
 #pragma unroll
                     for (int i = 0; i < 4; ++i) {
-                        float t = ok ? fmaf(y[i], sc[i], sh[i]) : 0.f;
+                        float t = ok ? fmaf(y[i], scu[i], shu[i]) : 0.f;
                         _Float16 hh = (_Float16)t;
                         hi[i] = hh;
                         lo[i] = (_Float16)(t - (float)hh);
@@ -386,25 +515,36 @@
     float fs[4] = {0.f, 0.f, 0.f, 0.f}, fq[4] = {0.f, 0.f, 0.f, 0.f};
     float mmn[4] = {INFINITY, INFINITY, INFINITY, INFINITY}, mmx[4] = {-INFINITY, -INFINITY, -INFINITY, -INFINITY};
     __syncthreads();
-    const int* rowtab = build_row_table<WM * 64, NTHR>(p, lds, tid, z0, y0, x0, boxN);
+    const int* rowtab = PK ? build_row_table_pk<WM * 64, NTHR>(p, lds, tid, nsub)
+                           : build_row_table<WM * 64, NTHR>(p, lds, tid, z0, y0, x0, boxN);
     __syncthreads();
+    float* const pk_tile = reinterpret_cast<float*>(lds + WM * 64 * 8);
     float* const ob = obase + (((int64_t)z0 * p.H + y0) * p.W + x0) * p.Cout + ntw * 64 + l32;
 #pragma unroll
     for (int mb = 0; mb < 2; ++mb) {
 #pragma unroll
         for (int ig = 0; ig < 4; ++ig) {
-            const int4 r4 = *reinterpret_cast<const int4*>(rowtab + wm * 64 + mb * 32 + row_perm(ig * 8 + khalf * 4));
+            const int q0 = wm * 64 + mb * 32 + row_perm(ig * 8 + khalf * 4);
+            const int4 r4 = *reinterpret_cast<const int4*>(rowtab + q0);
             const int rel[4] = {r4.x, r4.y, r4.z, r4.w};
+            int ae[4] = {0, 0, 0, 0};
+            if constexpr (PK) {
+                const int4 e4 = *reinterpret_cast<const int4*>(rowtab + WM * 64 + q0);
+                ae[0] = e4.x; ae[1] = e4.y; ae[2] = e4.z; ae[3] = e4.w;
+            }
 #pragma unroll
             for (int j = 0; j < 4; ++j) {
                 if (rel[j] < 0) continue;
                 float* orow = ob + (unsigned)rel[j];
+                const float dqr = PK ? ldexpf(1.0f, -(ae[j] + p.wexp)) : dq;
 #pragma unroll
                 for (int nb = 0; nb < 2; ++nb) {
-                    float r = acc[mb][nb][ig * 4 + j] * dq;
+                    float r = acc[mb][nb][ig * 4 + j] * dqr;
                     if (final_out) r = r >= 0.f ? r : r * p.slope;
                     orow[nb * 32] = r;
-                    if (want_rows) {
+                    if (PK && want_rows) {
+                        pk_tile[(q0 + j) * (64 * WN) + wn * 64 + nb * 32 + l32] = r;
+                    } else if (want_rows) {
                         fs[nb] += r; fq[nb] = fmaf(r, r, fq[nb]);
                         mmn[nb] = fminf(mmn[nb], r); mmx[nb] = fmaxf(mmx[nb], r);
                     }
@@ -412,7 +552,9 @@
             }
         }
     }
-    if (want_rows) {
+    if constexpr (PK) {
+        if (want_rows) store_moment_rows_pk<WM, WN, false>(p, lds, tid, smp, nsub, nt);
+    } else if (want_rows) {
         double ms[4], mq[4];
 #pragma unroll
         for (int j = 0; j < 4; ++j) { ms[j] = (double)fs[j]; mq[j] = (double)fq[j]; }
@@ -428,7 +570,7 @@
     }
 }
 
-template <int WM, int WN, int NPASS, int SP, int NSLOT>
+template <int WM, int WN, int NPASS, int SP, int NSLOT, bool PK = false>
 __global__ void __launch_bounds__(64 * WM * WN, 2) conv_mfma16(const ConvParams p) {
     constexpr int NTHR = 64 * WM * WN;
     constexpr int NW = WM * WN;
@@ -456,7 +598,11 @@
         bid = (xcd < r ? xcd * (q + 1) : r * (q + 1) + (xcd - r) * q) + idx;
     }
     int mt, nt, smp = 0;
-    if (p.S > 1) {
+    if constexpr (PK) {
+        mt = bid % p.nMt;
+        nt = bid / p.nMt;
+        smp = mt * p.P;
+    } else if (p.S > 1) {
         smp = bid % p.S;
         const int t = bid / p.S;
         nt = t % p.NT;
@@ -465,7 +611,8 @@
         mt = bid / p.NT;
         nt = bid - mt * p.NT;
     }
-    const int mtl = mt - smp * p.nMtS;
+    const int mtl = PK ? 0 : mt - smp * p.nMtS;
+    const int nsub = PK ? min(p.P, p.S - smp) : 1;
     const float* const pA = p.A + smp * p.sA;
     const float* const pB = p.B + smp * p.sB;
     const float* const pscale = p.scale + smp * p.saff;
@@ -479,6 +626,12 @@
     const int z0 = tz * p.TD, y0 = ty * p.TH, x0 = tx * p.TW;
     const int boxN = p.TD * p.TH * p.TW;
 
+    int* const pk_aexp = reinterpret_cast<int*>(lds + p.pk_tail);
+    float* const pk_aff = reinterpret_cast<float*>(pk_aexp + ((p.P + 3) & ~3));
+    if constexpr (PK) {
+        if (tid < p.P) pk_aexp[tid] = tid < nsub ? aexp_of_bound(pbound + tid * p.G, p.G) : 0;
+        __syncthreads();
+    }
     float bmax = 0.f;
     for (int g = 0; g < p.G; ++g) bmax = fmaxf(bmax, pbound[g]);
     int aexp = 0;
@@ -495,9 +648,12 @@
 #pragma unroll
     for (int rb = 0; rb < 4; ++rb) {
         int q = wm * 64 + rb * 16 + l16;
-        int d = 0, h = 0, w = 0;
-        if (q < boxN) box_coords(p, q, d, h, w);
-        int vox = (d * p.HT + h) * p.WT + w;
+        int d = 0, h = 0, w = 0, vbase = 0;
+        if constexpr (PK) {
+            const int sub = q / p.pvox;
+            if (sub < p.P) { box_coords(p, q - sub * p.pvox, d, h, w); vbase = sub * p.phalo; }
+        } else if (q < boxN) box_coords(p, q, d, h, w);
+        int vox = vbase + (d * p.HT + h) * p.WT + w;
         a_off[rb] = ((kg & 1) * NPL) * p.plane_stride + vox * 16;
     }
 
@@ -505,6 +661,7 @@
     const int n_el = p.nvox_lds * 4;
     const int q4 = tid & 3;
     int off[MAX_IT];
+    int ssubp[MAX_IT / 4] = {0, 0, 0};
     auto compute_offsets = [&](bool fromB) __attribute__((always_inline)) {
 #pragma unroll
         for (int it = 0; it < MAX_IT; ++it) {
@@ -512,15 +669,22 @@
             off[it] = -2;
             if (e < n_el) {
                 const int vox = e >> 2;
-                const int hz = vox / (p.HT * p.WT);
+                int hz = vox / (p.HT * p.WT);
                 const int rem = vox - hz * (p.HT * p.WT);
+                int sub = 0;
+                if constexpr (PK) {
+                    sub = hz / (p.D + 1);
+                    hz -= sub * (p.D + 1);
+                    ssubp[it >> 2] |= min(sub, nsub - 1) << ((it & 3) * 8);
+                }
                 const int hy = rem / p.WT;
                 const int hx = rem - hy * p.WT;
                 const int gz = z0 + hz - 1, gy = y0 + hy - 1, gx = x0 + hx - 1;
                 off[it] = -1;
-                if (gz >= 0 && gz < p.D && gy >= 0 && gy < p.H && gx >= 0 && gx < p.W) {
-                    if (fromB) off[it] = ((p.up.mapD[gz] * p.up.h + p.up.mapH[gy]) * p.up.w + p.up.mapW[gx]) * p.CB;
-                    else off[it] = ((gz * p.H + gy) * p.W + gx) * p.CA;
+                if (PK && sub >= nsub) {
+                } else if (gz >= 0 && gz < p.D && gy >= 0 && gy < p.H && gx >= 0 && gx < p.W) {
+                    if (!PK && fromB) off[it] = ((p.up.mapD[gz] * p.up.h + p.up.mapH[gy]) * p.up.w + p.up.mapW[gx]) * p.CB;
+                    else off[it] = (PK ? sub * (int)p.sA : 0) + ((gz * p.H + gy) * p.W + gx) * p.CA;
                 }
             }
         }
@@ -540,19 +704,26 @@
     const int ntw = nt * WN + wn;
     if (p.accum && p.splitk == 1) {
         const float inv_dq = ldexpf(1.0f, aexp + p.wexp);
-        const int* rowtab = build_row_table<WM * 64, NTHR>(p, lds, tid, z0, y0, x0, boxN);
+        const int* rowtab = PK ? build_row_table_pk<WM * 64, NTHR>(p, lds, tid, nsub)
+                               : build_row_table<WM * 64, NTHR>(p, lds, tid, z0, y0, x0, boxN);
         __syncthreads();
         const float* ib = pout + (((int64_t)z0 * p.H + y0) * p.W + x0) * p.Cout + ntw * 64 + l16;
 #pragma unroll
         for (int rb = 0; rb < 4; ++rb) {
             const int4 r4 = *reinterpret_cast<const int4*>(rowtab + wm * 64 + rb * 16 + kg * 4);
             const int rel[4] = {r4.x, r4.y, r4.z, r4.w};
+            int ae[4] = {0, 0, 0, 0};
+            if constexpr (PK) {
+                const int4 e4 = *reinterpret_cast<const int4*>(rowtab + WM * 64 + wm * 64 + rb * 16 + kg * 4);
+                ae[0] = e4.x; ae[1] = e4.y; ae[2] = e4.z; ae[3] = e4.w;
+            }
 #pragma unroll
             for (int i = 0; i < 4; ++i) {
                 if (rel[i] < 0) continue;
                 const float* orow = ib + (unsigned)rel[i];
-#pragma unroll
-                for (int cb = 0; cb < 4; ++cb) acc[rb][cb][i] = orow[cb * 16] * inv_dq;
+                const float idq = PK ? ldexpf(1.0f, ae[i] + p.wexp) : inv_dq;
+#pragma unroll
+                for (int cb = 0; cb < 4; ++cb) acc[rb][cb][i] = orow[cb * 16] * idq;
             }
         }
     }
@@ -594,6 +765,13 @@
         const float4 sh4 = *reinterpret_cast<const float4*>(pshift + c0 + q4 * 4);
         const float sc[4] = {sc4.x * a_scale, sc4.y * a_scale, sc4.z * a_scale, sc4.w * a_scale};
         const float sh[4] = {sh4.x * a_scale, sh4.y * a_scale, sh4.z * a_scale, sh4.w * a_scale};
+        if constexpr (PK) {
+            for (int i = tid; i < p.P * 32; i += NTHR) {
+                const int sb = min(i >> 5, nsub - 1), c = i & 15;
+                const float* row = ((i & 16) ? pshift : pscale) + sb * p.saff + c0;
+                pk_aff[i] = row[c] * ldexpf(1.0f, pk_aexp[sb]);
+            }
+        }
 
         __syncthreads();
 #pragma unroll
@@ -610,10 +788,20 @@
                 if (off[it0 + u] != -2) {
                     const bool ok = off[it0 + u] >= 0;
                     float y[4] = {v[u].x, v[u].y, v[u].z, v[u].w};
+                    float scu[4], shu[4];
+                    if constexpr (PK) {
+                        const float* af = pk_aff + ((ssubp[(it0 + u) >> 2] >> (((it0 + u) & 3) * 8)) & 255) * 32 + q4 * 4;
+                        const float4 a4 = *reinterpret_cast<const float4*>(af), b4 = *reinterpret_cast<const float4*>(af + 16);
+                        scu[0] = a4.x; scu[1] = a4.y; scu[2] = a4.z; scu[3] = a4.w;
+                        shu[0] = b4.x; shu[1] = b4.y; shu[2] = b4.z; shu[3] = b4.w;
+                    } else {
+#pragma unroll
+                        for (int i = 0; i < 4; ++i) { scu[i] = sc[i]; shu[i] = sh[i]; }
+                    }
                     half4 hi, lo;
 #pragma unroll
                     for (int i = 0; i < 4; ++i) {
-                        float t = ok ? fmaf(y[i], sc[i], sh[i]) : 0.f;
+                        float t = ok ? fmaf(y[i], scu[i], shu[i]) : 0.f;
                         _Float16 hh = (_Float16)t;
                         hi[i] = hh;
                         lo[i] = (_Float16)(t - (float)hh);
@@ -685,30 +873,43 @@
     float fs[4] = {0.f, 0.f, 0.f, 0.f}, fq[4] = {0.f, 0.f, 0.f, 0.f};
     float mmn[4] = {INFINITY, INFINITY, INFINITY, INFINITY}, mmx[4] = {-INFINITY, -INFINITY, -INFINITY, -INFINITY};
     __syncthreads();
-    const int* rowtab = build_row_table<WM * 64, NTHR>(p, lds, tid, z0, y0, x0, boxN);
+    const int* rowtab = PK ? build_row_table_pk<WM * 64, NTHR>(p, lds, tid, nsub)
+                           : build_row_table<WM * 64, NTHR>(p, lds, tid, z0, y0, x0, boxN);
     __syncthreads();
+    float* const pk_tile = reinterpret_cast<float*>(lds + WM * 64 * 8);
     float* const ob = obase + (((int64_t)z0 * p.H + y0) * p.W + x0) * p.Cout + ntw * 64 + l16;
 #pragma unroll
     for (int rb = 0; rb < 4; ++rb) {
-        const int4 r4 = *reinterpret_cast<const int4*>(rowtab + wm * 64 + rb * 16 + kg * 4);
+        const int q0 = wm * 64 + rb * 16 + kg * 4;
+        const int4 r4 = *reinterpret_cast<const int4*>(rowtab + q0);
         const int rel[4] = {r4.x, r4.y, r4.z, r4.w};
+        int ae[4] = {0, 0, 0, 0};
+        if constexpr (PK) {
+            const int4 e4 = *reinterpret_cast<const int4*>(rowtab + WM * 64 + q0);
+            ae[0] = e4.x; ae[1] = e4.y; ae[2] = e4.z; ae[3] = e4.w;
+        }
 #pragma unroll
         for (int i = 0; i < 4; ++i) {
             if (rel[i] < 0) continue;
             float* orow = ob + (unsigned)rel[i];
+            const float dqr = PK ? ldexpf(1.0f, -(ae[i] + p.wexp)) : dq;
 #pragma unroll
             for (int cb = 0; cb < 4; ++cb) {
-                float r = acc[rb][cb][i] * dq;
+                float r = acc[rb][cb][i] * dqr;
                 if (final_out) r = r >= 0.f ? r : r * p.slope;
                 orow[cb * 16] = r;
-                if (want_rows) {
+                if (PK && want_rows) {
+                    pk_tile[(q0 + i) * (64 * WN) + wn * 64 + cb * 16 + l16] = r;
+                } else if (want_rows) {
                     fs[cb] += r; fq[cb] = fmaf(r, r, fq[cb]);
                     mmn[cb] = fminf(mmn[cb], r); mmx[cb] = fmaxf(mmx[cb], r);
                 }
             }
         }
     }
-    if (want_rows) {
+    if constexpr (PK) {
+        if (want_rows) store_moment_rows_pk<WM, WN, true>(p, lds, tid, smp, nsub, nt);
+    } else if (want_rows) {
         double ms[4], mq[4];
 #pragma unroll
         for (int j = 0; j < 4; ++j) { ms[j] = (double)fs[j]; mq[j] = (double)fq[j]; }
@@ -1289,6 +1490,47 @@
                          dim3(64 * WM * WN), smem, st, p);
 }
 
+int launch_packed(const ConvParams& p, int passes, int ver, bool wm4, dim3 grid, size_t smem, hipStream_t st) {
+    static bool attr = false;
+    if (const int rc = bfm_raise_lds_limit(
+            attr,
+            {bfm_kernel(&conv_mfma<4, 1, 3, nslot_for(1), true>), bfm_kernel(&conv_mfma<4, 1, 1, nslot_for(1), true>),
+             bfm_kernel(&conv_mfma<2, 2, 3, nslot_for(2), true>), bfm_kernel(&conv_mfma<2, 2, 1, nslot_for(2), true>),
+             bfm_kernel(&conv_mfma16<4, 1, 3, 2, 2, true>), bfm_kernel(&conv_mfma16<4, 1, 1, 2, 2, true>),
+             bfm_kernel(&conv_mfma16<2, 2, 3, 1, 3, true>), bfm_kernel(&conv_mfma16<2, 2, 1, 1, 3, true>)},
+            LDS_LIMIT))
+        return rc;
+    if (ver == 2) {
+        if (wm4) bfm_launch_by_passes(passes, conv_mfma16<4, 1, 3, 2, 2, true>, conv_mfma16<4, 1, 1, 2, 2, true>, grid, dim3(256), smem, st, p);
+        else bfm_launch_by_passes(passes, conv_mfma16<2, 2, 3, 1, 3, true>, conv_mfma16<2, 2, 1, 1, 3, true>, grid, dim3(256), smem, st, p);
+    } else {
+        if (wm4) bfm_launch_by_passes(passes, conv_mfma<4, 1, 3, nslot_for(1), true>, conv_mfma<4, 1, 1, nslot_for(1), true>, grid, dim3(256), smem, st, p);
+        else bfm_launch_by_passes(passes, conv_mfma<2, 2, 3, nslot_for(2), true>, conv_mfma<2, 2, 1, nslot_for(2), true>, grid, dim3(256), smem, st, p);
+    }
+    return BFM_OK;
+}
+
+int pack_factor(const HostPlan& hp, int S, int CB, int D, int H, int W, int64_t sA, int64_t sO, int npl) {
+    static const bool pack_on = [] { const char* e = getenv("BFM_PACK_M"); return !(e && e[0] == '0'); }();
+    if (!pack_on || S < 2 || CB > 0 || (hp.ver != 0 && hp.ver != 2)) return 1;
+    if (hp.TD < D || hp.TH < H || hp.TW < W) return 1;
+    const int ROWS = hp.WM * 64;
+    const int64_t nvox = (int64_t)D * H * W;
+    if (nvox > ROWS / 2) return 1;
+    const int plane = (H + 2) * (W + 2);
+    int64_t P = std::min<int64_t>(S, ROWS / nvox);
+    P = std::min<int64_t>(P, (12 * 64 * hp.WM * hp.WN / 4 / plane - 1) / (D + 1));
+    P = std::min<int64_t>(P, 0x7fffffffLL / std::max<int64_t>(1, std::max(sA, sO)));
+    for (; P >= 2; --P) {
+        const int staged = ((int)P * (D + 1) + 1) * plane;
+        const int ps = hp.ver == 2 ? plane_stride16_for(staged) : plane_stride_for(staged);
+        const size_t loop = (size_t)2 * npl * ps + (hp.ver == 2 ? ring16_bytes(hp.WN) : ring_bytes(hp.WN));
+        const size_t epi = (size_t)ROWS * 8 + (size_t)P * nvox * 64 * hp.WN * sizeof(float);
+        if (std::max(loop, epi) + 16 * bfm_cdiv((int)P, 4) + 128 * (size_t)P <= (size_t)LDS_LIMIT) break;
+    }
+    return P >= 2 ? (int)P : 1;
+}
+
 }
 
 extern "C" size_t bfm_pack_conv_weights_mfma_bytes(int Cin, int Cout) {
@@ -1426,6 +1668,16 @@
 
 extern "C" size_t bfm_conv3x3x3_mfma_batch_workspace(int Cin, int Cout, int S, int D, int H, int W, int splitk) {
     return (size_t)(S < 1 ? 1 : S) * bfm_conv3x3x3_mfma_workspace(Cin, Cout, D, H, W, splitk);
+}
+
+extern "C" int bfm_conv3x3x3_mfma_batch_pack(int Cin, int Cout, int S, int D, int H, int W, const int* cfg, int passes,
+                                             int two_sources) {
+    if (!cfg || Cin <= 0 || Cout <= 0 || S < 1 || D <= 0 || H <= 0 || W <= 0 || (passes != 1 && passes != 3)) return 1;
+    const HostPlan hp{cfg[0], cfg[1], cfg[2], cfg[3], cfg[4], cfg[5], cfg[6]};
+    const bool wg_ok = (hp.WM == 4 && hp.WN == 1) || (hp.WM == 2 && hp.WN == 2);
+    if (!wg_ok || hp.TD < 1 || hp.TH < 1 || hp.TW < 1 || hp.TD * hp.TH * hp.TW > hp.WM * 64) return 1;
+    const int64_t nvox = (int64_t)D * H * W;
+    return pack_factor(hp, S, two_sources ? 1 : 0, D, H, W, nvox * Cin, nvox * Cout, passes == 3 ? 2 : 1);
 }
 
 extern "C" int bfm_conv3x3x3_mfma_batch(const float* A, int CA, const float* B, int CB, int S, int D, int H, int W,
@@ -1488,18 +1740,32 @@
     if (p.splitk > p.KCN) p.splitk = p.KCN;
     p.kc_per_split = bfm_cdiv(p.KCN, p.splitk);
     p.splitk = bfm_cdiv(p.KCN, p.kc_per_split);
-    p.nvox_lds = (hp.TD + 2) * p.HT * p.WT;
+    const int npl = passes == 3 ? 2 : 1;
+    const int64_t nvox = (int64_t)D * H * W;
+    const int P = pack_factor(hp, S, CB, D, H, W, nvox * CA, nvox * Cout, npl);
+    size_t pk_epi = 0;
+    if (P > 1) {
+        p.P = P; p.pvox = (int)nvox; p.phalo = (D + 1) * (H + 2) * (W + 2);
+        p.oTH = hp.TH; p.oTW = hp.TW; p.oboxN = hp.TD * hp.TH * hp.TW;
+        hp.TD = D; hp.TH = H; hp.TW = W;
+        p.TD = D; p.TH = H; p.TW = W; p.HT = H + 2; p.WT = W + 2;
+        pk_epi = (size_t)hp.WM * 64 * 8 + (size_t)P * nvox * 64 * hp.WN * sizeof(float);
+    }
+    p.nvox_lds = (P > 1 ? P * (D + 1) + 1 : hp.TD + 2) * p.HT * p.WT;
     p.plane_stride = hp.ver == 2 ? plane_stride16_for(p.nvox_lds) : plane_stride_for(p.nvox_lds);
     p.tw_shift = is_pow2(hp.TW) ? ilog2(hp.TW) : -1;
     p.thw_shift = is_pow2(hp.TH * hp.TW) ? ilog2(hp.TH * hp.TW) : -1;
-    const int npl = passes == 3 ? 2 : 1;
-    const size_t smem = hp.ver == 1 ? (size_t)ws_smem(npl, p.plane_stride, hp.WN)
-                        : hp.ver == 2 ? (size_t)2 * npl * p.plane_stride + ring16_bytes(hp.WN)
-                                      : (size_t)2 * npl * p.plane_stride + ring_bytes(hp.WN);
+    size_t smem = hp.ver == 1 ? (size_t)ws_smem(npl, p.plane_stride, hp.WN)
+                  : hp.ver == 2 ? (size_t)2 * npl * p.plane_stride + ring16_bytes(hp.WN)
+                                : (size_t)2 * npl * p.plane_stride + ring_bytes(hp.WN);
+    if (P > 1) {
+        smem = (std::max(smem, pk_epi) + 15) / 16 * 16;
+        p.pk_tail = (int)smem;
+        smem += (size_t)16 * bfm_cdiv(P, 4) + (size_t)128 * P;
+    }
     if (smem > (size_t)(hp.ver == 1 ? LDS_LIMIT_WS : LDS_LIMIT)) return BFM_E_SHAPE;
     if (hp.ver < 0 || hp.ver > 2) return BFM_E_ARG;
     if (p.nvox_lds * 4 > 12 * 64 * hp.WM * hp.WN) return BFM_E_SHAPE;
-    const int64_t nvox = (int64_t)D * H * W;
     p.sA = nvox * CA;
     p.sB = CB > 0 ? (int64_t)up->d * up->h * up->w * CB : 0;
     p.sO = nvox * Cout;
@@ -1519,6 +1785,7 @@
         if (!rows.carve(moment_rows, (size_t)p.nMt * Cout)) return BFM_E_ARG;
         rows.into(p);
     }
+    if (P > 1) p.nMt = bfm_cdiv(S, P);
 #ifdef BFM_MFMA_ABLATE
     if (const char* e = getenv("BFM_MFMA_ABL")) p.abl = atoi(e);
 #endif
@@ -1533,7 +1800,9 @@
     }
     dim3 grid(gx, (unsigned)p.splitk);
     hipStream_t st = bfm_s(stream);
-    if (hp.ver == 2) {
+    if (P > 1) {
+        if (const int rc = launch_packed(p, passes, hp.ver, hp.WM == 4, grid, smem, st)) return rc;
+    } else if (hp.ver == 2) {
         launch16(p, passes, hp.WM == 4, grid, smem, st);
     } else if (hp.ver == 1) {
         if (const int rc = hp.WM == 4 ? launch_ws<4, 1>(p, passes, grid, smem, st) : launch_ws<2, 2>(p, passes, grid, smem, st))
diff --git a/include/brainfm_hip.h b/include/brainfm_hip.h
--- a/include/brainfm_hip.h
+++ b/include/brainfm_hip.h
@@ -90,6 +90,8 @@
                           int G, const void* wpacked, int wexp, int Cout, float slope, int passes, const int* cfg,
                           float* out, void* workspace, size_t workspace_bytes, void* moment_rows ,
                           bfm_stream_t stream);
+int bfm_conv3x3x3_mfma_batch_pack(int Cin, int Cout, int S, int D, int H, int W, const int* cfg, int passes,
+                                  int two_sources);
 size_t bfm_conv3x3x3_mfma_batch_workspace(int Cin, int Cout, int S, int D, int H, int W, int splitk);
 int bfm_conv3x3x3_mfma_batch(const float* A, int CA, const float* B, int CB, int S, int D, int H, int W,
                              const bfm_upsample_t* up, const float* scale, const float* shift, const float* bound, int G,
```

After: 201.9 million voxels/s (median of 6 runs). Within noise of the previous version (+0.8%).
